# cavelandiah/BBMap

Hardware: AMD Instinct MI355X
Metric: aligned_reads_per_sec (higher is better)
Workload: dtype int32

## Files before the change

bbmap_amd/csrc/mapper_host.hip:

```cpp
#include <hip/hip_runtime.h>

#include <algorithm>
#include <cstdlib>
#include <cstring>
#include <new>
#include <thread>
#include <vector>

#include "mapper_ctx.h"

using namespace bbmapper;

extern "C" int bbmap_default_config_profile(int32_t profile, bbmap_config *c) {
    if (!c || (profile != BBIDX_PROFILE_BBMAP && profile != BBIDX_PROFILE_PACBIO)) return bbfail(BBMAP_E_ARG, "bbmap_default_config: bad argument");
    memset(c, 0, sizeof *c);
    c->paired = 0; c->max_reads = 0; c->max_sites = 32;
    c->extraPadding = 10; c->maxPairDist = 32000; c->averagePairDist = 100; c->maxRescueDist = 1200; c->maxRescueMismatches = 32;
    c->maxTrimSitesToRetain = 800; c->trimList = 1; c->doRescue = 1; c->clearzone3 = 800; c->fastCols = 0; c->jobsPerRead = 0;
    c->finalStage = profile == BBIDX_PROFILE_BBMAP ? 1 : 0;
    if (profile == BBIDX_PROFILE_PACBIO) {
        c->max_read_len = 6016; c->minRatio = 0.46f; c->slowAlignPadding = 8; c->slowRescuePadding = 16; c->tipSearchDist = 15;
        c->alignColumns = 7600; c->msaMaxColumns = 7600;
    } else {
        c->max_read_len = 150; c->minRatio = 0.56f; c->slowAlignPadding = 4; c->slowRescuePadding = 8; c->tipSearchDist = 100;
        c->alignColumns = 3000; c->msaMaxColumns = 3000;
    }
    c->reserved[3] = profile;
    return BBMAP_OK;
}
extern "C" int bbmap_default_config(bbmap_config *c) { return bbmap_default_config_profile(BBIDX_PROFILE_BBMAP, c); }

extern "C" void bbmap_destroy(bbmap_ctx *c) {
    if (!c) return;
    (void)hipSetDevice(c->cfg.device);
    for (void *p : c->allocs) (void)hipFree(p);
    if (c->h_counters) (void)hipHostFree(c->h_counters);
    if (c->tierThread.joinable()) c->tierThread.join();
    if (c->tier) bbmap_destroy(c->tier);
    bbidx_launch_free(&c->probeLs);
    for (DevBuf &b : c->buf) b.release();
    if (c->hostStream) (void)hipStreamDestroy(c->hostStream);
    if (c->tierStream) (void)hipStreamDestroy(c->tierStream);
    if (c->dpStream) (void)hipStreamDestroy(c->dpStream);
    if (c->evFork) (void)hipEventDestroy(c->evFork);
    if (c->evJoin) (void)hipEventDestroy(c->evJoin);
    if (c->ownsMsa && c->msaGapped && c->msaGapped != c->msa) bbmsa_destroy(c->msaGapped);
    if (c->ownsMsa && c->msa) bbmsa_destroy(c->msa);
    for (hipEvent_t e : c->ev) if (e) (void)hipEventDestroy(e);
    delete c;
}

static int create_impl(bbidx_ctx *index, const bbmap_config *cfg, bbmap_ctx *parent, bbmap_ctx **out) {
    if (!index || !cfg || !out) return bbfail(BBMAP_E_ARG, "bbmap_create: null argument");
    *out = nullptr;
    const int profile = cfg->reserved[3];
    if (profile != BBIDX_PROFILE_BBMAP && profile != BBIDX_PROFILE_PACBIO) return bbfail(BBMAP_E_ARG, "bbmap_create: unknown profile (bbmap_config.reserved[3])");
    if (profile != index->dev.p.profile) return bbfail(BBMAP_E_ARG, "bbmap_create: the index was built for the other profile (BBIDX_PROFILE_*)");
    const bool pacbio = profile == BBIDX_PROFILE_PACBIO;
    if (cfg->max_reads < 1 || cfg->max_read_len < 1 || cfg->max_read_len > (pacbio ? BBIDX_PACBIO_MAX_READ_LEN : 600))
        return bbfail(BBMAP_E_ARG, "bbmap_create: max_reads >= 1 and max_read_len in 1..600 (1..6016 for BBIDX_PROFILE_PACBIO)");
    if (cfg->max_sites < 1 || cfg->max_sites > BBMAP_MAX_SITES_LIMIT) return bbfail(BBMAP_E_ARG, "bbmap_create: max_sites must be 1..4096");
    if (cfg->paired && (cfg->max_reads & 1)) return bbfail(BBMAP_E_ARG, "bbmap_create: paired mode takes an even number of reads");
    if (cfg->msaMaxColumns < 64 || cfg->msaMaxColumns > (pacbio ? 8192 : 4096)) return bbfail(BBMAP_E_ARG, "bbmap_create: msaMaxColumns must be 64..4096 (..8192 for BBIDX_PROFILE_PACBIO)");
    if (cfg->device != index->device) return bbfail(BBMAP_E_ARG, "bbmap_create: the index lives on another device");
    BBHIP(hipSetDevice(cfg->device));
    bbmap_ctx *c = new (std::nothrow) bbmap_ctx();
    if (!c) return bbfail(BBMAP_E_NOMEM, "bbmap_create: out of host memory");
    c->cfg = *cfg; c->index = index;
    int rc = BBMAP_OK;
    auto bail = [&](int code) { bbmap_destroy(c); return code; };
    if ((rc = bbidx_launch_init(index, &c->probeLs)) != BBMAP_OK) return bail(rc);
    Settings &S = c->S;
    const float R = cfg->minRatio;
    S.minRatio = R;
    { const float a = R * .80f, b = 1.0f - ((1.0f - R) * 1.4f); S.ratioPaired = a > b ? a : b; }
    { const float a = R * .60f, b = 1.0f - ((1.0f - R) * 1.8f); S.ratioPreRescue = a > b ? a : b; }
    S.slowAlignPadding = cfg->slowAlignPadding; S.slowRescuePadding = cfg->slowRescuePadding; S.extraPadding = cfg->extraPadding;
    S.tipSearchDist = cfg->tipSearchDist; S.maxPairDist = cfg->maxPairDist; S.averagePairDist = cfg->averagePairDist;
    S.maxRescueDist = cfg->maxRescueDist; S.maxRescueMismatches = cfg->maxRescueMismatches; S.maxTrimSitesToRetain = cfg->maxTrimSitesToRetain;
    S.trimList = cfg->trimList; S.doRescue = cfg->doRescue; S.alignColumns = cfg->alignColumns; S.clearzone3 = cfg->clearzone3;
    S.maxIndel = index->dev.p.maxIndel; S.paired = cfg->paired; S.rescueSkip = 0;
    if (pacbio) { S.ptsMatch = 90; S.ptsMatch2 = 100; S.ptsSub = -137; S.ptsSub2 = -49; S.ptsSub3 = -25; S.impDelta = -305; }
    else { S.ptsMatch = 70; S.ptsMatch2 = 100; S.ptsSub = -127; S.ptsSub2 = -51; S.ptsSub3 = -25; S.impDelta = -495; }
    S.clearzone1e = 2 * S.ptsMatch2 - S.ptsMatch - S.ptsSub + 1;
    S.msaMaxColumns = cfg->msaMaxColumns;
    if (pacbio) { S.ptsSubR = -157; S.ptsIns = -205; S.ptsIns2 = -42; S.ptsIns3 = -23; S.ptsIns4 = -8; S.ptsDel = -292; S.ptsDel2 = -37; S.ptsDel3 = -17; S.ptsDel4 = -2; }
    else { S.ptsSubR = -147; S.ptsIns = -395; S.ptsIns2 = -39; S.ptsIns3 = -23; S.ptsIns4 = -8; S.ptsDel = -472; S.ptsDel2 = -33; S.ptsDel3 = -9; S.ptsDel4 = -1; }
    S.ptsDel5 = -1; S.ptsGap = -2;
    if (pacbio && (cfg->finalStage < 0 || cfg->finalStage > 2)) return bail(bbfail(BBMAP_E_ARG, "bbmap_create: finalStage must be 0, 1 or 2"));
    S.finalStage = cfg->finalStage ? 1 : 0;
    S.finalPolicy = (pacbio && cfg->finalStage == 1) ? 1 : 0;
    {
        const float rP = S.finalPolicy ? 1.5f : 1.6f, r1 = S.finalPolicy ? 2.2f : 2.0f, r1b = S.finalPolicy ? 2.8f : 2.6f, r1c = S.finalPolicy ? 4.8f : 4.6f;
        const float m2 = (float)S.ptsMatch2;
        S.czP = (int)(rP * m2); S.cz1 = (int)(r1 * m2); S.cz1b = (int)(r1b * m2); S.cz1c = (int)(r1c * m2);
        S.czLimit1e = 40;
    }
    index->dev.p.quitAfterTwoPerfects = cfg->paired ? 0 : 1;
    S.expLimit = (cfg->alignColumns * 17) / 20 - (2 * (cfg->slowAlignPadding + 10));
    const int maxRows = ((cfg->max_read_len + 31) / 32) * 32;
    c->maxRows = maxRows;
    bbmsa_config mc; memset(&mc, 0, sizeof mc);
    mc.device = cfg->device; mc.maxRows = maxRows;
    bbmsa_config gc;
    if (pacbio) {
        mc.maxRows = cfg->max_read_len + 4 > 6100 ? 6100 : cfg->max_read_len + 4;
        c->maxRows = mc.maxRows;
        mc.maxColumns = cfg->msaMaxColumns;
        mc.reserved[2] = BBMSA_SCHEME_9PACBIO;
        gc = mc;
        c->plainColumns = mc.maxColumns;
        if (parent) { c->msa = parent->msa; c->msaGapped = parent->msaGapped; c->ownsMsa = false; }
        else {
            c->ownsMsa = true;
            if ((rc = bbmsa_create(&mc, &c->msa)) != BBMAP_OK) return bail(rc);
            c->msaGapped = c->msa;
        }
    } else {
        mc.maxColumns = cfg->fastCols > 0 ? cfg->fastCols : 256;
        if (mc.maxColumns > cfg->msaMaxColumns) mc.maxColumns = cfg->msaMaxColumns;
        c->plainColumns = mc.maxColumns;
        gc = mc;
        gc.maxColumns = cfg->msaMaxColumns;
        gc.reserved[0] = 32; gc.reserved[1] = 640 < gc.maxColumns ? 640 : gc.maxColumns;
        if (const char *e = getenv("BBMAP_G2_LANES")) { if (*e) gc.reserved[0] = atoi(e); }
        if (const char *e = getenv("BBMAP_G2_COLS")) { if (*e) gc.reserved[1] = atoi(e) < gc.maxColumns ? atoi(e) : gc.maxColumns; }
        (void)parent;
        c->ownsMsa = true;
        if ((rc = bbmsa_create(&mc, &c->msa)) != BBMAP_OK) return bail(rc);
        if ((rc = bbmsa_create(&gc, &c->msaGapped)) != BBMAP_OK) return bail(rc);
    }
    const long long n = cfg->max_reads;
    const int cap = cfg->max_sites;
    c->narrowMinJobs = getenv("BBMAP_NARROW_MIN_JOBS") ? atoll(getenv("BBMAP_NARROW_MIN_JOBS")) : 32768;
    c->sortWide = !(getenv("BBMAP_SORT_WIDE") && atoi(getenv("BBMAP_SORT_WIDE")) == 0);
    if (!pacbio) {
        const long long lat = getenv("BBMAP_LATENCY_JOBS") ? atoll(getenv("BBMAP_LATENCY_JOBS")) : 4096;
        if ((rc = bbmsa_set_latency_jobs(c->msa, lat)) != BBMAP_OK) return bail(rc);
        if (c->msaGapped != c->msa && (rc = bbmsa_set_latency_jobs(c->msaGapped, lat)) != BBMAP_OK) return bail(rc);
    }
    const int jpr = cfg->jobsPerRead > 0 ? cfg->jobsPerRead : 3;
    c->jobCap = n * jpr + 1024;
    c->gjobCap = parent ? n * 16 + 4096 : (n * jpr) / 24 + 4096;
    if (cfg->jobsPerRead < 0) c->jobCap = c->gjobCap = -(long long)cfg->jobsPerRead;
    c->rescCap = parent ? n * 64 + 1024 : n * 2 + 1024;
    c->matchStride = ((maxRows + c->plainColumns + 15) / 16) * 16;
    c->gmatchStride = ((maxRows + gc.maxColumns + 2 + 128 * 8 + 15) / 16) * 16;
#define DA(ptr, count) if ((rc = dalloc(c, &(ptr), (size_t)(count))) != BBMAP_OK) return bail(rc)
    DA(c->d_psites, n * cap); DA(c->d_pnsites, n);
    DA(c->d_ms, n * cap); DA(c->d_mcount, n); DA(c->d_near, n);
    DA(c->d_slow, n);
    DA(c->d_active[0], n); DA(c->d_active[1], n);
    DA(c->d_counters, CNT_WORDS);
    DA(c->d_jobs, c->jobCap); DA(c->d_jinfo, c->jobCap); DA(c->d_results, c->jobCap); DA(c->d_match, c->jobCap * c->matchStride);
    DA(c->d_gjobs, c->gjobCap); DA(c->d_ggaps, c->gjobCap); DA(c->d_ginfo, c->gjobCap); DA(c->d_gresults, c->gjobCap); DA(c->d_gmatch, c->gjobCap * c->gmatchStride);
    DA(c->d_rjobs, c->rescCap); DA(c->d_rinfo, c->rescCap); DA(c->d_rres, c->rescCap); DA(c->d_rsite, c->rescCap);
    DA(c->d_pres, n / 2 + 1);
    if (S.finalStage) {
        c->poolUnits = (n * (long long)(3 * (cfg->max_read_len + 16)) + 65536) / 4;
        if (const char *e = getenv("BBMAP_FINAL_POOL_UNITS")) { if (*e && atoll(e) >= 64) c->poolUnits = atoll(e); }
        DA(c->d_fin, n); DA(c->d_final, n); DA(c->d_pool, c->poolUnits * 4);
    }
    const int nch = index->dev.nchroms;
    DA(c->d_chromMin, nch + 1); DA(c->d_chromOff, nch + 1);
#undef DA
    c->d_chromArr = index->dev.chromArr; c->d_chromArrLen = index->dev.chromArrLen;
    {
        std::vector<const uint8_t *> hc((size_t)nch + 1);
        if (hipMemcpy(hc.data(), index->dev.chromArr, sizeof(void *) * hc.size(), hipMemcpyDeviceToHost) != hipSuccess) return bail(bbfail(BBMAP_E_HIP, "bbmap_create: reading the chromosome table failed"));
        c->refsBase = hc[1];
        std::vector<long long> off((size_t)nch + 1, 0);
        for (int i = 1; i <= nch; i++) off[(size_t)i] = (long long)(hc[(size_t)i] - hc[1]);
        if (hipMemcpy(c->d_chromOff, off.data(), 8 * off.size(), hipMemcpyHostToDevice) != hipSuccess) return bail(bbfail(BBMAP_E_HIP, "bbmap_create: upload failed"));
        if (hipMemset(c->d_chromMin, 0, 4 * ((size_t)nch + 1)) != hipSuccess) return bail(bbfail(BBMAP_E_HIP, "bbmap_create: memset failed"));
    }
    if (hipHostMalloc((void **)&c->h_counters, CNT_WORDS * 4) != hipSuccess) return bail(bbfail(BBMAP_E_NOMEM, "bbmap_create: pinned allocation failed"));
    for (hipEvent_t &e : c->ev) if (hipEventCreate(&e) != hipSuccess) return bail(bbfail(BBMAP_E_HIP, "bbmap_create: hipEventCreate failed"));
    if (!getenv("BBMAP_SERIAL_DP") && !pacbio) {
        if (hipStreamCreateWithFlags(&c->dpStream, hipStreamNonBlocking) != hipSuccess || hipEventCreateWithFlags(&c->evFork, hipEventDisableTiming) != hipSuccess ||
            hipEventCreateWithFlags(&c->evJoin, hipEventDisableTiming) != hipSuccess) return bail(bbfail(BBMAP_E_HIP, "bbmap_create: stream / event creation failed"));
    }
    *out = c;
    return BBMAP_OK;
}

extern "C" int bbmap_create(bbidx_ctx *index, const bbmap_config *cfg, bbmap_ctx **out) {
    bbmap_ctx *c = nullptr;
    BBTRY(create_impl(index, cfg, nullptr, &c));
    if (cfg->reserved[1] >= 0) {
        bbmap_config tc = *cfg;
        long long tn = cfg->reserved[1] > 0 ? cfg->reserved[1] : 4096;
        if (tn > cfg->max_reads) tn = cfg->max_reads;
        if (cfg->paired) tn &= ~1ll;
        tc.max_reads = (int32_t)tn;
        tc.max_sites = cfg->reserved[2] > 0 ? cfg->reserved[2] : 1024;
        tc.jobsPerRead = 128;
        tc.reserved[1] = -1;
        if (tn >= (cfg->paired ? 2 : 1) && tc.max_sites > cfg->max_sites) {
            const int rc = create_impl(index, &tc, c, &c->tier);
            if (rc != BBMAP_OK) { bbmap_destroy(c); return rc; }
            const long long units = cfg->paired ? cfg->max_reads / 2 : cfg->max_reads;
            if (dalloc(c, &c->d_tierUnits, (size_t)units + 1) != BBMAP_OK || dalloc(c, &c->d_tierReads, (size_t)tn) != BBMAP_OK ||
                dalloc(c, &c->d_tierReadIds, (size_t)tn) != BBMAP_OK) { bbmap_destroy(c); return BBMAP_E_NOMEM; }
            if (hipStreamCreateWithFlags(&c->tierStream, hipStreamNonBlocking) != hipSuccess) { bbmap_destroy(c); return bbfail(BBMAP_E_HIP, "bbmap_create: hipStreamCreate failed"); }
        }
    }
    *out = c;
    return BBMAP_OK;
}

static int read_counters(bbmap_ctx *c, hipStream_t stream) {
    BBHIP(hipMemcpyAsync(c->h_counters, c->d_counters, CNT_WORDS * 4, hipMemcpyDeviceToHost, stream));
    BBHIP(hipStreamSynchronize(stream));
    return BBMAP_OK;
}

template <class T> static int regrow(bbmap_ctx *c, hipStream_t stream, T **p, size_t oldCount, size_t newCount, std::vector<void *> &dead) {
    void *d = nullptr;
    if (hipMalloc(&d, (newCount ? newCount : 1) * sizeof(T)) != hipSuccess) return bbfail(BBMAP_E_NOMEM, "bbmap_map_batch_device: growing a fill log failed (device memory)");
    if (oldCount) BBHIP(hipMemcpyAsync(d, *p, oldCount * sizeof(T), hipMemcpyDeviceToDevice, stream));
    for (void *&q : c->allocs) if (q == (void *)*p) q = d;
    dead.push_back((void *)*p);
    *p = (T *)d;
    return BBMAP_OK;
}
struct DeadArrays {
    hipStream_t stream; std::vector<void *> v;
    explicit DeadArrays(hipStream_t s) : stream(s) {}
    ~DeadArrays() { if (!v.empty()) { (void)hipStreamSynchronize(stream); for (void *q : v) (void)hipFree(q); } }
};
static int grow_logs(bbmap_ctx *c, hipStream_t stream, Dev &D, long long needJobs, long long needGapped, long long usedJobs, long long usedGapped) {
    DeadArrays guard(stream);
    std::vector<void *> &dead = guard.v;
    if (needJobs > c->jobCap) {
        long long nc = c->jobCap * 2; if (nc < needJobs) nc = needJobs + needJobs / 4 + 1024;
        BBTRY(regrow(c, stream, &c->d_jobs, (size_t)usedJobs, (size_t)nc, dead));
        BBTRY(regrow(c, stream, &c->d_jinfo, (size_t)usedJobs, (size_t)nc, dead));
        BBTRY(regrow(c, stream, &c->d_results, (size_t)usedJobs, (size_t)nc, dead));
        BBTRY(regrow(c, stream, &c->d_match, (size_t)usedJobs * c->matchStride, (size_t)nc * c->matchStride, dead));
        c->jobCap = nc;
    }
    if (needGapped > c->gjobCap) {
        long long nc = c->gjobCap * 2; if (nc < needGapped) nc = needGapped + needGapped / 4 + 1024;
        BBTRY(regrow(c, stream, &c->d_gjobs, (size_t)usedGapped, (size_t)nc, dead));
        BBTRY(regrow(c, stream, &c->d_ggaps, (size_t)usedGapped, (size_t)nc, dead));
        BBTRY(regrow(c, stream, &c->d_ginfo, (size_t)usedGapped, (size_t)nc, dead));
        BBTRY(regrow(c, stream, &c->d_gresults, (size_t)usedGapped, (size_t)nc, dead));
        BBTRY(regrow(c, stream, &c->d_gmatch, (size_t)usedGapped * c->gmatchStride, (size_t)nc * c->gmatchStride, dead));
        c->gjobCap = nc;
    }
    c->h_counters[CNT_STAGE_FILLS] = (unsigned)usedJobs; c->h_counters[CNT_STAGE_GAPPED] = (unsigned)usedGapped;
    BBHIP(hipMemcpyAsync(c->d_counters + CNT_FILLS, c->h_counters + CNT_STAGE_FILLS, 8, hipMemcpyHostToDevice, stream));
    BBHIP(hipStreamSynchronize(stream));
    D.jobs = c->d_jobs; D.jinfo = c->d_jinfo; D.results = c->d_results; D.match = c->d_match; D.jobCap = c->jobCap;
    D.gjobs = c->d_gjobs; D.ggaps = c->d_ggaps; D.ginfo = c->d_ginfo; D.gresults = c->d_gresults; D.gmatch = c->d_gmatch; D.gjobCap = c->gjobCap;
    c->stats.log_growths += 1.0f;
    return BBMAP_OK;
}

static int run_fills(bbmap_ctx *c, hipStream_t stream, const uint8_t *bases, long long jobBase, long long nNew, long long gBase, long long gNew,
                     bool finalStage = false) {
    bbmsa_use_narrow(c->msa, !finalStage && nNew >= c->narrowMinJobs);
    bbmsa_sort_by_width(c->msa, false);
    if (c->msaGapped != c->msa) { bbmsa_use_narrow(c->msaGapped, false); bbmsa_sort_by_width(c->msaGapped, c->sortWide); }
    hipStream_t gs = (c->dpStream && nNew > 0) ? c->dpStream : stream;
    if (gNew > 0) {
        if (gs != stream) { BBHIP(hipEventRecord(c->evFork, stream)); BBHIP(hipStreamWaitEvent(gs, c->evFork, 0)); }
        BBTRY(bbmsa_align_gapped_batch_device(c->msaGapped, gs, gNew, c->d_gjobs + gBase, c->d_ggaps + gBase, bases, c->refsBase,
                                             c->d_gresults + gBase, c->d_gmatch + gBase * c->gmatchStride, c->gmatchStride));
        if (gs != stream) { BBHIP(hipEventRecord(c->evJoin, gs)); if (nNew > 0) BBTRY(bbmsa_wait_first_pass(c->msaGapped, stream)); }
    }
    if (nNew > 0)
        BBTRY(bbmsa_align_batch_device(c->msa, stream, nNew, c->d_jobs + jobBase, bases, c->refsBase, c->d_results + jobBase,
                                      c->d_match + jobBase * c->matchStride, c->matchStride));
    const int r1 = nNew > 0 ? bbmsa_last_route_flags(c->msa) : 0;
    const int r2 = gNew > 0 ? bbmsa_last_route_flags(c->msaGapped) : 0;
    c->stats.dp_narrow_launches += (r1 & 1) + (r2 & 1);
    c->stats.dp_sorted_launches += ((r1 >> 1) & 1) + ((r2 >> 1) & 1);
    if (gNew > 0 && gs != stream) BBHIP(hipStreamWaitEvent(stream, c->evJoin, 0));
    return BBMAP_OK;
}

static void add_dp_ms(bbmap_ctx *c, bool plain, bool gapped) {
    float k3[3];
    if (plain && bbmsa_last_kernel_ms3(c->msa, k3) == BBMAP_OK) { c->stats.ms_dp_narrow += k3[0]; c->stats.ms_dp_wave += k3[1]; c->stats.ms_dp_generic += k3[2];
                                                                 if (k3[1] > c->stats.ms_dp_wave_max) c->stats.ms_dp_wave_max = k3[1]; }
    if (gapped && c->msaGapped != c->msa && bbmsa_last_kernel_ms3(c->msaGapped, k3) == BBMAP_OK) c->stats.ms_dp_gapped += k3[0] + k3[1] + k3[2];
    static const bool show = getenv("BBMAP_DP_COUNTS") != nullptr;
    if (show) {
        int64_t n4[4];
        if (plain && bbmsa_last_counts(c->msa, n4) == BBMAP_OK)
            fprintf(stderr, "dp counts plain : narrow finished %lld, narrow handed on %lld, wavefront list %lld, to the wide/generic pass %lld\n",
                    (long long)n4[0], (long long)n4[1], (long long)n4[2], (long long)n4[3]);
        if (gapped && bbmsa_last_counts(c->msaGapped, n4) == BBMAP_OK)
            fprintf(stderr, "dp counts second: narrow finished %lld, narrow handed on %lld, wavefront list %lld, to the wide/generic pass %lld\n",
                    (long long)n4[0], (long long)n4[1], (long long)n4[2], (long long)n4[3]);
    }
}

static void tier_start_async(bbmap_ctx *c, long long found);

struct Rounds {
    bool finalStage;
    long long jobBase, gBase;
    long long nActive;
    int cur = 0;
    bool first = true, ranPlain = false, ranGapped = false;
};
template <class K> static int round_begin(bbmap_ctx *c, hipStream_t stream, Dev &D, Rounds &R, K kernel) {
    BBHIP(hipMemsetAsync(c->d_counters + CNT_NEXT_ACTIVE, 0, 4, stream));
    if (R.finalStage) {
        BBHIP(hipMemsetAsync(c->d_counters + CNT_POOL_AT_FAILURE, 0xff, 4, stream));
        BBHIP(hipMemsetAsync(c->d_counters + CNT_POOL_FAILED, 0, 4, stream));
    }
    D.activeIn = R.first ? nullptr : c->d_active[R.cur]; D.nActiveIn = (int)R.nActive; D.activeOut = c->d_active[1 - R.cur];
    BBTRY(launch<128>(kernel, R.nActive, stream, D));
    return read_counters(c, stream);
}
static int round_end(bbmap_ctx *c, hipStream_t stream, Dev &D, Rounds &R, const uint8_t *bases) {
    add_dp_ms(c, R.ranPlain, R.ranGapped);
    const long long asked = c->h_counters[CNT_FILLS], gasked = c->h_counters[CNT_GAPPED_FILLS];
    const long long total = asked < c->jobCap ? asked : c->jobCap, gtotal = gasked < c->gjobCap ? gasked : c->gjobCap;
    BBTRY(run_fills(c, stream, bases, R.jobBase, total - R.jobBase, R.gBase, gtotal - R.gBase, R.finalStage));
    R.ranPlain = total > R.jobBase; R.ranGapped = gtotal > R.gBase;
    R.jobBase = total; R.gBase = gtotal;
    if (asked > c->jobCap || gasked > c->gjobCap) BBTRY(grow_logs(c, stream, D, asked, gasked, total, gtotal));
    R.nActive = c->h_counters[CNT_NEXT_ACTIVE];
    R.cur = 1 - R.cur; R.first = false;
    return BBMAP_OK;
}

static int grow_pool(bbmap_ctx *c, hipStream_t stream, Dev &D, long long used, long long units, bool setCounter) {
    if (units > 0x7ffffff0LL) return bbfail(BBMAP_E_NOMEM, "bbmap_map_batch_device: the final stage's match strings exceed 8 GB; map smaller batches");
    DeadArrays guard(stream);
    BBTRY(regrow(c, stream, &c->d_pool, (size_t)used * 4, (size_t)units * 4, guard.v));
    if (setCounter) {
        c->h_counters[CNT_STAGE_POOL] = (unsigned)used;
        BBHIP(hipMemcpyAsync(c->d_counters + CNT_POOL_UNITS, c->h_counters + CNT_STAGE_POOL, 4, hipMemcpyHostToDevice, stream));
    }
    BBHIP(hipStreamSynchronize(stream));
    c->poolUnits = units; D.pool = c->d_pool; D.poolUnits = units;
    return BBMAP_OK;
}

static int run_final_stage(bbmap_ctx *c, hipStream_t stream, Dev &D, int64_t n_reads, const uint8_t *bases, long long jobBase, long long gBase,
                           long long &finalRounds, long long &finalLocal) {
    const long long units = c->cfg.paired ? n_reads / 2 : n_reads;
    const unsigned *h = c->h_counters;
    D.fin = c->d_fin; D.finalOut = c->d_final; D.pool = c->d_pool; D.poolUnits = c->poolUnits;
    D.match = c->d_match; D.gmatch = c->d_gmatch; D.matchStride = c->matchStride; D.gmatchStride = c->gmatchStride;
    BBTRY(launch<128>(final_begin_kernel, units, stream, D));
    Rounds R; R.finalStage = true; R.jobBase = jobBase; R.gBase = gBase; R.nActive = n_reads;
    for (int round = 0; R.nActive > 0; round++) {
        if (round > 64 * c->cfg.max_sites + 64) return bbfail(BBMAP_E_HIP, "bbmap_map_batch_device: the final stage does not come to an end (internal error)");
        BBTRY(round_begin(c, stream, D, R, final_round_kernel));
        BBTRY(round_end(c, stream, D, R, bases));
        if (h[CNT_POOL_FAILED] > 0) {
            const long long used = h[CNT_POOL_AT_FAILURE];
            long long nu = c->poolUnits * 2, need = used + ((long long)h[CNT_POOL_UNITS] - used) * 2 + 65536;
            if (nu < need) nu = need;
            BBTRY(grow_pool(c, stream, D, used, nu, true));
        }
        finalRounds++;
    }
    BBHIP(hipStreamSynchronize(stream));
    add_dp_ms(c, R.ranPlain, R.ranGapped);
    BBHIP(hipMemsetAsync(c->d_counters + CNT_LOCAL_READS, 0, 8, stream));
    BBTRY(launch<128>(final_end_kernel, units, stream, D));
    BBTRY(read_counters(c, stream));
    finalLocal = h[CNT_LOCAL_READS];
    const long long used = h[CNT_POOL_UNITS], local = h[CNT_LOCAL_UNITS];
    if (used + local + 64 > c->poolUnits) BBTRY(grow_pool(c, stream, D, used, used + local + 65536, false));
    BBTRY(launch<128>(final_local_kernel, units, stream, D));
    return BBMAP_OK;
}


static void fill_dev(bbmap_ctx *c, Dev &D, int64_t n_reads, const bbidx_read *reads, uint8_t *bases, int64_t minus_delta) {
    memset(&D, 0, sizeof D);
    D.S = c->S; D.reads = reads; D.bases = bases; D.minusDelta = minus_delta; D.nreads = n_reads;
    D.chromArr = c->d_chromArr; D.chromArrLen = c->d_chromArrLen; D.refsBase = c->refsBase;
    D.psites = c->d_psites; D.pnsites = c->d_pnsites; D.maxSites = c->cfg.max_sites;
    D.ms = c->d_ms; D.mcount = c->d_mcount; D.cap = c->cfg.max_sites; D.nearArr = c->d_near; D.slow = c->d_slow;
    D.counters = c->d_counters; D.plainColumns = c->plainColumns; D.fillAhead = c->cfg.reserved[0] ? 0 : 1;
    D.jobs = c->d_jobs; D.jinfo = c->d_jinfo; D.results = c->d_results; D.jobCap = c->jobCap;
    D.gjobs = c->d_gjobs; D.ggaps = c->d_ggaps; D.ginfo = c->d_ginfo; D.gresults = c->d_gresults; D.gjobCap = c->gjobCap;
    D.rjobs = c->d_rjobs; D.rinfo = c->d_rinfo; D.rres = c->d_rres; D.pres = c->d_pres; D.rescCap = c->rescCap; D.rsite = c->d_rsite;
    if (c->index->scafFilter) D.scaf = c->index->scaf;
}

static int finish_stats(bbmap_ctx *c, hipStream_t stream, bool whole, long long fillsBefore, long long finalRounds, long long finalLocal) {
    BBHIP(hipEventRecord(c->ev[EV_FINAL_END], stream));
    BBTRY(read_counters(c, stream));
    const unsigned *h = c->h_counters;
    const hipEvent_t *ev = c->ev;
    c->poolUsed = 4ll * h[CNT_POOL_UNITS];
    c->nJobs = h[CNT_FILLS]; c->nGapped = h[CNT_GAPPED_FILLS];
    c->finalFills = c->S.finalStage ? (c->nJobs + c->nGapped) - fillsBefore : 0;
    bbmap_stats &st = c->stats;
    st.fills = c->nJobs; st.gapped_fills = c->nGapped;
    (void)hipEventElapsedTime(&st.ms_final, ev[EV_RESCUE_END], ev[EV_FINAL_END]);
    if (whole) {
        st.reads_overflowed = h[CNT_OVERFLOWED]; st.reads_without_site = h[CNT_NO_SITE];
        st.refills = h[CNT_REFILLS]; st.rescue_fills = h[CNT_RESCUE_FILLS]; st.fills_dropped = h[CNT_FILLS_DROPPED];
        st.sites_cross_scaffold = h[CNT_CROSS_SCAFFOLD];
        (void)hipEventElapsedTime(&st.ms_probe, ev[EV_START], ev[EV_PROBE_END]);
        (void)hipEventElapsedTime(&st.ms_begin, ev[EV_PROBE_END], ev[EV_BEGIN_END]);
        (void)hipEventElapsedTime(&st.ms_score, ev[EV_BEGIN_END], ev[EV_SCORE_END]);
        (void)hipEventElapsedTime(&st.ms_slow, ev[EV_SCORE_END], ev[EV_SLOW_END]);
        (void)hipEventElapsedTime(&st.ms_finish, ev[EV_SLOW_END], ev[EV_FINISH_END]);
        (void)hipEventElapsedTime(&st.ms_rescue, ev[EV_FINISH_END], ev[EV_RESCUE_END]);
        (void)hipEventElapsedTime(&st.ms_total, ev[EV_START], ev[EV_FINAL_END]);
    } else st.ms_total = st.ms_final;
    st.final_fills = c->finalFills; st.final_rounds = finalRounds; st.final_local = finalLocal;
    return BBMAP_OK;
}

static int map_records(bbmap_ctx *c, hipStream_t stream, int64_t n_reads, const bbidx_read *reads, uint8_t *bases,
                       int64_t minus_delta, const int8_t *baseScores, const int32_t *keyinfo, bool writeRc) {
    memset(&c->stats, 0, sizeof c->stats);
    c->stats.reads = n_reads;
    BBHIP(hipMemsetAsync(c->d_counters, 0, CNT_WORDS * 4, stream));
    BBHIP(hipEventRecord(c->ev[EV_START], stream));
    BBTRY(bbidx_find_batch_device_with(c->index, &c->probeLs, stream, n_reads, reads, bases, baseScores, keyinfo, c->d_psites, c->cfg.max_sites,
                                      c->d_pnsites, writeRc ? bases + minus_delta : nullptr));
    if (writeRc) BBTRY(launch<128>(revcomp_unprobed_kernel, n_reads, stream, reads, (long long)n_reads, (int)c->index->dev.p.k, (const uint8_t *)bases, bases + minus_delta));
    BBHIP(hipEventRecord(c->ev[EV_PROBE_END], stream));
    Dev D;
    fill_dev(c, D, n_reads, reads, bases, minus_delta);
    const long long units = c->cfg.paired ? n_reads / 2 : n_reads;
    BBTRY(launch<128>(begin_kernel, units, stream, D));
    if (c->tier) {
        BBTRY(launch<128>(collect_overflow_kernel, units, stream, c->d_mcount, units, c->cfg.paired, c->d_tierUnits, c->d_counters + CNT_TIER_FOUND));
    }
    BBHIP(hipEventRecord(c->ev[EV_BEGIN_END], stream));
    BBTRY(launch<128>(score_kernel, n_reads, stream, D));
    BBHIP(hipEventRecord(c->ev[EV_SCORE_END], stream));
    Rounds R; R.finalStage = false; R.jobBase = R.gBase = 0; R.nActive = n_reads;
    for (int round = 0; R.nActive > 0 && round < 4 * c->cfg.max_sites + 4; round++) {
        BBTRY(round_begin(c, stream, D, R, slow_round_kernel));
        if (round == 0) {
            float pms = 0; long long ps[5];
            if (writeRc && bbidx_last_stats_with(c->index, &c->probeLs, (int64_t *)ps, &pms) == BBMAP_OK) for (int i = 0; i < 5; i++) c->stats.probe_stats[i] = ps[i];
            c->overAfterBegin = c->h_counters[CNT_OVERFLOWED];
            if (c->tier && c->h_counters[CNT_TIER_FOUND] > 0 && c->tier->msa != c->msa) tier_start_async(c, c->h_counters[CNT_TIER_FOUND]);
        }
        BBTRY(round_end(c, stream, D, R, bases));
        c->stats.rounds++;
    }
    long long jobBase = R.jobBase, gBase = R.gBase;
    BBHIP(hipEventRecord(c->ev[EV_SLOW_END], stream));
    BBTRY(launch<128>(finish_kernel, n_reads, stream, D));
    BBHIP(hipEventRecord(c->ev[EV_FINISH_END], stream));
    if (c->cfg.paired && c->cfg.doRescue) {
        const long long pairs = n_reads / 2;
        for (int pass = 0; pass < 2; pass++) {
            D.pass = pass;
            BBHIP(hipMemsetAsync(c->d_counters + CNT_RESCUE_SEARCHES, 0, 4, stream));
            BBTRY(launch<128>(rescue_plan_kernel, pairs, stream, D));
            BBTRY(read_counters(c, stream));
            const long long nsearch = c->h_counters[CNT_RESCUE_SEARCHES];
            if (nsearch > c->rescCap) return bbfail(BBMAP_E_NOMEM, "bbmap_map_batch_device: rescue list full");
            c->stats.rescue_scans += nsearch;
            if (nsearch == 0) {
                BBTRY(launch<128>(rescue_finish_kernel, pairs, stream, D));
                continue;
            }
            hipEvent_t q0 = c->ev[EV_QUICK_BEGIN], q1 = c->ev[EV_QUICK_END];
            BBHIP(hipEventRecord(q0, stream));
            BBTRY(bbpipe_quick_rescue_device(stream, nsearch, c->d_rjobs, bases, (const int64_t *)c->d_chromOff, c->d_chromArrLen, c->d_chromMin, c->refsBase,
                                            c->d_rres, c->S.ptsMatch, c->S.ptsMatch2, 1, 100));
            BBHIP(hipEventRecord(q1, stream));
            if (jobBase + nsearch > c->jobCap || gBase + nsearch > c->gjobCap) BBTRY(grow_logs(c, stream, D, jobBase + nsearch, gBase + nsearch, jobBase, gBase));
            BBTRY(launch<128>(rescue_prep_kernel, pairs, stream, D));
            BBTRY(read_counters(c, stream));
            { float ms = 0; if (hipEventElapsedTime(&ms, q0, q1) == hipSuccess) c->stats.ms_quick_rescue += ms; }
            const long long total = c->h_counters[CNT_FILLS], gtotal = c->h_counters[CNT_GAPPED_FILLS];
            if (total > c->jobCap || gtotal > c->gjobCap) return bbfail(BBMAP_E_HIP, "bbmap_map_batch_device: rescue fills beyond the reserved log entries (internal error)");
            BBTRY(run_fills(c, stream, bases, jobBase, total - jobBase, gBase, gtotal - gBase));
            const bool ranPlain = total > jobBase, ranGapped = gtotal > gBase;
            jobBase = total; gBase = gtotal;
            BBTRY(launch<128>(rescue_finish_kernel, pairs, stream, D));
            BBHIP(hipStreamSynchronize(stream));
            add_dp_ms(c, ranPlain, ranGapped);
        }
    }
    BBHIP(hipEventRecord(c->ev[EV_RESCUE_END], stream));
    c->finalFills = 0; c->poolUsed = 0;
    long long finalRounds = 0, finalLocal = 0;
    if (c->S.finalStage) BBTRY(run_final_stage(c, stream, D, n_reads, bases, jobBase, gBase, finalRounds, finalLocal));
    BBTRY(finish_stats(c, stream, true, jobBase + gBase, finalRounds, finalLocal));
    c->ran = true;
    return BBMAP_OK;
}

static int tier_pass(bbmap_ctx *c, hipStream_t s, long long found) {
    bbmap_ctx *t = c->tier;
    const bbmap_ctx::BatchArgs &B = c->batch;
    const int paired = c->cfg.paired;
    c->tierReads = 0; t->ran = false;
    std::vector<int> ids((size_t)found);
    BBHIP(hipMemcpyAsync(ids.data(), c->d_tierUnits, 4 * (size_t)found, hipMemcpyDeviceToHost, s));
    BBHIP(hipStreamSynchronize(s));
    std::sort(ids.begin(), ids.end());
    const long long room = paired ? t->cfg.max_reads / 2 : t->cfg.max_reads;
    const long long take = found < room ? found : room;
    BBHIP(hipMemcpyAsync(c->d_tierUnits, ids.data(), 4 * (size_t)take, hipMemcpyHostToDevice, s));
    BBTRY(launch<128>(gather_reads_kernel, take, s, B.reads, c->d_tierUnits, (int)take, paired, c->d_tierReads, c->d_tierReadIds));
    BBHIP(hipStreamSynchronize(s));
    const long long tn = paired ? 2 * take : take;
    BBTRY(map_records(t, s, tn, c->d_tierReads, B.bases, B.minus_delta, B.baseScores, B.keyinfo, false));
    c->tierReads = tn;
    return BBMAP_OK;
}

static void tier_start_async(bbmap_ctx *c, long long found) {
    c->tierStarted = true; c->tierRc = BBMAP_OK; c->tierErr[0] = 0;
    c->tierThread = std::thread([c, found]() {
        int rc = hipSetDevice(c->cfg.device) == hipSuccess ? BBMAP_OK : BBMAP_E_HIP;
        if (rc == BBMAP_OK) rc = tier_pass(c, c->tierStream, found);
        if (rc != BBMAP_OK) { snprintf(c->tierErr, sizeof c->tierErr, "overflow tier: %s", bbmap_last_error()); }
        c->tierRc = rc;
    });
}

static int tier_finish(bbmap_ctx *c, hipStream_t stream) {
    bbmap_ctx *t = c->tier;
    const long long tn = c->tierReads;
    if (tn == 0) return BBMAP_OK;
    BBHIP(hipMemsetAsync(c->d_counters + CNT_TIER_RESOLVED, 0, 4, stream));
    BBTRY(launch<128>(mark_tier_kernel, tn, stream, c->d_mcount, t->d_mcount, c->d_tierReadIds, (int)tn, c->d_counters + CNT_TIER_RESOLVED));
    BBTRY(read_counters(c, stream));
    bbmap_stats &st = c->stats; const bbmap_stats &ts = t->stats;
    st.reads_reprobed = tn;
    st.reads_overflowed -= (long long)c->h_counters[CNT_TIER_RESOLVED];
    st.reads_without_site += ts.reads_without_site;
    st.fills += ts.fills; st.gapped_fills += ts.gapped_fills; st.refills += ts.refills; st.rescue_scans += ts.rescue_scans;
    st.rescue_fills += ts.rescue_fills; st.fills_dropped += ts.fills_dropped;
    st.final_fills += ts.final_fills; st.final_local += ts.final_local;
    st.dp_narrow_launches += ts.dp_narrow_launches; st.dp_sorted_launches += ts.dp_sorted_launches;
    st.sites_cross_scaffold += ts.sites_cross_scaffold;
    if (getenv("BBMAP_TIER_DEBUG"))
        fprintf(stderr, "[bbmap tier] reads %lld: probe %.2f begin %.2f score %.2f slow %.2f (rounds %lld) finish %.2f rescue %.2f total %.2f\n",
                tn, ts.ms_probe, ts.ms_begin, ts.ms_score, ts.ms_slow, (long long)ts.rounds, ts.ms_finish, ts.ms_rescue, ts.ms_total);
    return BBMAP_OK;
}

static int rescue_skip_rule(bbmap_ctx *c, bool *skip) {
    *skip = false;
    if (!c->d_runStats) return BBMAP_OK;
    bbmap_runstats rs;
    BBHIP(hipStreamSynchronize(c->statsStream));
    BBHIP(hipMemcpy(&rs, c->d_runStats, sizeof rs, hipMemcpyDeviceToHost));
    *skip = rs.mappedRetained2 > 1000 && rs.numMated * 20LL < rs.mappedRetained2;
    return BBMAP_OK;
}

static int adapt_after_batch(bbmap_ctx *c, hipStream_t stream) {
    if (!(c->adaptive & BBMAP_ADAPT_INSERT_LENGTH)) return BBMAP_OK;
    bbmap_runstats rs;
    BBHIP(hipMemcpyAsync(&rs, c->d_runStats, sizeof rs, hipMemcpyDeviceToHost, stream));
    BBHIP(hipStreamSynchronize(stream));
    const bool heldPaired = rs.numMated > c->numMatedSeen;
    c->numMatedSeen = rs.numMated;
    if (rs.numMated > 1000 && heldPaired) {
        volatile float sum = (float)rs.innerLengthSum, cnt = (float)rs.numMated;
        const float q = sum * 1.0f / cnt;
        const int v = (int)q;
        if (v >= 0) BBTRY(bbmap_set_average_pair_dist(c, v));
    }
    return BBMAP_OK;
}

extern "C" int bbmap_get_adaptive_state(bbmap_ctx *c, int32_t *averagePairDist, int32_t *rescueSkipped) {
    if (!c) return bbfail(BBMAP_E_ARG, "bbmap_get_adaptive_state: null context");
    if (averagePairDist) *averagePairDist = c->cfg.averagePairDist;
    if (rescueSkipped) {
        bool skip = false;
        if (c->adaptive & BBMAP_ADAPT_RESCUE_SKIP) { BBHIP(hipSetDevice(c->cfg.device)); BBTRY(rescue_skip_rule(c, &skip)); }
        *rescueSkipped = skip ? 1 : 0;
    }
    return BBMAP_OK;
}

static int map_batch_device(bbmap_ctx *c, hipStream_t stream, int64_t n_reads, const bbidx_read *reads, uint8_t *bases,
                            int64_t minus_delta, const int8_t *baseScores, const int32_t *keyinfo) {
    c->batch = {n_reads, reads, bases, minus_delta, baseScores, keyinfo};
    c->tierStarted = false; c->tierReads = 0;
    if (c->tier) c->tier->ran = false;
    const int rc = map_records(c, stream, n_reads, reads, bases, minus_delta, baseScores, keyinfo, true);
    hipEvent_t e0 = c->ev[EV_TIER_BEGIN], e1 = c->ev[EV_TIER_END];
    if (c->tierStarted) {
        c->tierThread.join();
        if (rc == BBMAP_OK && c->tierRc != BBMAP_OK) return bbfail(c->tierRc, "%s", c->tierErr);
    }
    BBTRY(rc);
    if (c->tier) BBHIP(hipEventRecord(e0, stream));
    if (!c->tier || c->stats.reads_overflowed == 0) return BBMAP_OK;
    if (c->stats.reads_overflowed > c->overAfterBegin || !c->tierStarted) {
        const long long units = c->cfg.paired ? n_reads / 2 : n_reads;
            BBHIP(hipMemsetAsync(c->d_counters + CNT_TIER_FOUND, 0, 4, stream));
        BBTRY(launch<128>(collect_overflow_kernel, units, stream, c->d_mcount, units, c->cfg.paired, c->d_tierUnits, c->d_counters + CNT_TIER_FOUND));
        BBTRY(read_counters(c, stream));
        if (c->h_counters[CNT_TIER_FOUND] > 0) BBTRY(tier_pass(c, stream, c->h_counters[CNT_TIER_FOUND]));
    }
    BBTRY(tier_finish(c, stream));
    BBHIP(hipEventRecord(e1, stream));
    BBHIP(hipStreamSynchronize(stream));
    (void)hipEventElapsedTime(&c->stats.ms_overflow, e0, e1);
    c->stats.ms_total += c->stats.ms_overflow;
    return BBMAP_OK;
}

extern "C" int bbmap_map_batch_device(bbmap_ctx *c, void *stream_, int64_t n_reads, const bbidx_read *reads, uint8_t *bases,
                                      int64_t minus_delta, const int8_t *baseScores, const int32_t *keyinfo) {
    if (!c) return bbfail(BBMAP_E_ARG, "bbmap_map_batch_device: null context");
    if (n_reads < 0 || n_reads > c->cfg.max_reads) return bbfail(BBMAP_E_ARG, "bbmap_map_batch_device: more reads than the context was made for");
    if (c->cfg.paired && (n_reads & 1)) return bbfail(BBMAP_E_ARG, "bbmap_map_batch_device: paired mode takes an even number of reads");
    if (n_reads == 0) { c->ran = false; c->truthNext = nullptr; return BBMAP_OK; }
    if (!reads || !bases || !baseScores || !keyinfo) return bbfail(BBMAP_E_ARG, "bbmap_map_batch_device: null buffer");
    hipStream_t stream = (hipStream_t)stream_;
    BBHIP(hipSetDevice(c->cfg.device));
    c->statsCounted = false;
    const bbmap_truth *truth = c->truthNext;
    c->truthNext = nullptr;
    bool skip = false;
    if (c->adaptive & BBMAP_ADAPT_RESCUE_SKIP) BBTRY(rescue_skip_rule(c, &skip));
    c->S.rescueSkip = skip ? 1 : 0;
    if (c->tier) c->tier->S.rescueSkip = c->S.rescueSkip;
    BBTRY(map_batch_device(c, stream, n_reads, reads, bases, minus_delta, baseScores, keyinfo));
    if (c->adaptive && c->S.finalStage) {
        BBTRY(bbmap_add_run_stats(c, stream, truth));
        BBTRY(adapt_after_batch(c, stream));
    }
    return BBMAP_OK;
}

extern "C" int bbmap_final_batch_device(bbmap_ctx *c, void *stream_, int64_t n_reads, const bbidx_read *reads, uint8_t *bases, int64_t minus_delta,
                                        const bbmap_msite *sites, const int32_t *nsites) {
    if (!c) return bbfail(BBMAP_E_ARG, "bbmap_final_batch_device: null context");
    if (!c->S.finalStage) return bbfail(BBMAP_E_ARG, "bbmap_final_batch_device: the context was created without the final stage");
    if (n_reads < 1 || n_reads > c->cfg.max_reads || (c->cfg.paired && (n_reads & 1))) return bbfail(BBMAP_E_ARG, "bbmap_final_batch_device: bad read count");
    if (!reads || !bases || !sites || !nsites) return bbfail(BBMAP_E_ARG, "bbmap_final_batch_device: null buffer");
    hipStream_t stream = (hipStream_t)stream_;
    BBHIP(hipSetDevice(c->cfg.device));
    c->tierStarted = false; c->tierReads = 0;
    if (c->tier) c->tier->ran = false;
    c->statsCounted = false;
    memset(&c->stats, 0, sizeof c->stats);
    c->stats.reads = n_reads;
    c->batch = {n_reads, reads, bases, minus_delta, nullptr, nullptr};
    BBHIP(hipMemsetAsync(c->d_counters, 0, CNT_WORDS * 4, stream));
    BBHIP(hipMemsetAsync(c->d_slow, 0, sizeof(SlowState) * (size_t)n_reads, stream));
    BBHIP(hipMemcpyAsync(c->d_ms, sites, sizeof(bbmap_msite) * (size_t)n_reads * (size_t)c->cfg.max_sites, hipMemcpyDeviceToDevice, stream));
    BBHIP(hipMemcpyAsync(c->d_mcount, nsites, 4 * (size_t)n_reads, hipMemcpyDeviceToDevice, stream));
    BBHIP(hipEventRecord(c->ev[EV_RESCUE_END], stream));
    Dev D;
    fill_dev(c, D, n_reads, reads, bases, minus_delta);
    long long finalRounds = 0, finalLocal = 0;
    BBTRY(run_final_stage(c, stream, D, n_reads, bases, 0, 0, finalRounds, finalLocal));
    BBTRY(finish_stats(c, stream, false, 0, finalRounds, finalLocal));
    c->ran = true;
    return BBMAP_OK;
}
```

bbmap_amd/csrc/msa_common.h:

```cpp
#pragma once
#include <hip/hip_runtime.h>
#include <stdint.h>
#include "bbmap_amd.h"

namespace bbmsa {

constexpr int kScoreOffset = 11;
constexpr int kTimeMask = 0x7FF;
constexpr int kScoreMask = (int)0xFFFFF800;
constexpr int kMaxTime = 2047;

#define BBMSA_PT(x) ((x) * 2048)
constexpr int P_MATCH = BBMSA_PT(70), P_MATCH2 = BBMSA_PT(100);
constexpr int P_SUB = BBMSA_PT(-127), P_SUBR = BBMSA_PT(-147), P_SUB2 = BBMSA_PT(-51), P_SUB3 = BBMSA_PT(-25);
constexpr int P_INS = BBMSA_PT(-395), P_INS2 = BBMSA_PT(-39), P_INS3 = BBMSA_PT(-23), P_INS4 = BBMSA_PT(-8);
constexpr int P_DEL = BBMSA_PT(-472), P_DEL2 = BBMSA_PT(-33), P_DEL3 = BBMSA_PT(-9), P_DEL4 = BBMSA_PT(-1),
              P_DEL5 = BBMSA_PT(-1);
constexpr int P_DEL_REF_N = BBMSA_PT(-10), P_GAP = BBMSA_PT(-2);
constexpr int kBadOff = (-(((1 << 20) - 1) - 2000) - 1) * 2048;
constexpr int kMinOffScore = (-(((1 << 20) - 1) - 2000)) * 2048;
constexpr int kNegInf = -(1 << 30);
constexpr int kGapLen = 128;

constexpr int kTableLen = 3072;
__host__ __device__ inline int lds_table_ints(int tableLen) { return 2 * tableLen + 320; }

__host__ __device__ inline int lds_job_ints(int fastCols, int tmpBytes) { return (fastCols + 2) + ((fastCols + 2 + 3) >> 2) + ((tmpBytes + 3) >> 2); }

__host__ __device__ inline int calc_del_off(int len) {
    if (len <= 0) return 0;
    int s = P_DEL;
    if (len > 80) { s += ((len - 80 + 3) / 4) * P_DEL5; len = 80; }
    if (len > 20) { s += (len - 20) * P_DEL4; len = 20; }
    if (len > 5) { s += (len - 5) * P_DEL3; len = 5; }
    if (len > 1) s += (len - 1) * P_DEL2;
    return s;
}
__host__ __device__ inline int calc_ins_cum_off(int len) {
    if (len <= 0) return 0;
    long long s = P_INS;
    int n = len;
    if (n > 20) { s += (long long)(n - 20) * P_INS4; n = 20; }
    if (n > 5) { s += (long long)(n - 5) * P_INS3; n = 5; }
    if (n > 1) s += (long long)(n - 1) * P_INS2;
    return s < kMinOffScore ? kMinOffScore : (int)s;
}

__host__ __device__ inline bool fully_defined(int b) {
    const int u = b & ~32;
    return b < 128 && (u == 'A' || u == 'C' || u == 'G' || u == 'T' || u == 'U');
}

struct Scheme11ts {
    static constexpr int OFF = kScoreOffset, TMASK = kTimeMask, SMASK = kScoreMask, MAXT = kMaxTime;
    static constexpr int MATCH = P_MATCH, MATCH2 = P_MATCH2, SUB = P_SUB, SUBR = P_SUBR, SUB2 = P_SUB2, SUB3 = P_SUB3;
    static constexpr int INS = P_INS, INS2 = P_INS2, INS3 = P_INS3, INS4 = P_INS4;
    static constexpr int DEL = P_DEL, DEL2 = P_DEL2, DEL3 = P_DEL3, DEL4 = P_DEL4, DEL5 = P_DEL5;
    static constexpr int DEL_REF_N = P_DEL_REF_N, GAP = P_GAP;
    static constexpr int BAR_I1 = 2, BAR_D1 = 3;
    static constexpr int BADOFF = kBadOff;
    __host__ __device__ static inline int del_off(int len) { return calc_del_off(len); }
    __host__ __device__ static inline int ins_cum_off(int len) { return calc_ins_cum_off(len); }
    __host__ __device__ static inline int col0(int row) { return calc_ins_cum_off(row); }
};
struct Scheme9PacBio {
    static constexpr int OFF = 9, TMASK = 0x1FF, SMASK = (int)0xFFFFFE00, MAXT = 511;
#define BBMSA_PB(x) ((x) * 512)
    static constexpr int MATCH = BBMSA_PB(90), MATCH2 = BBMSA_PB(100);
    static constexpr int SUB = BBMSA_PB(-137), SUBR = BBMSA_PB(-157), SUB2 = BBMSA_PB(-49), SUB3 = BBMSA_PB(-25);
    static constexpr int INS = BBMSA_PB(-205), INS2 = BBMSA_PB(-42), INS3 = BBMSA_PB(-23), INS4 = BBMSA_PB(-8);
    static constexpr int DEL = BBMSA_PB(-292), DEL2 = BBMSA_PB(-37), DEL3 = BBMSA_PB(-17), DEL4 = BBMSA_PB(-2), DEL5 = BBMSA_PB(-1);
    static constexpr int DEL_REF_N = BBMSA_PB(-10), GAP = BBMSA_PB(-2);
    static constexpr int BAR_I1 = 1, BAR_D1 = 1;
    static constexpr int BADOFF = (-(((1 << 22) - 1) - 2000) - 1) * 512;
#undef BBMSA_PB
    __host__ __device__ static inline int del_off(int len) {
        if (len <= 0) return 0;
        int s = DEL;
        if (len > 80) { s += ((len - 80 + 3) / 4) * DEL5; len = 80; }
        if (len > 20) { s += (len - 20) * DEL4; len = 20; }
        if (len > 5) { s += (len - 5) * DEL3; len = 5; }
        if (len > 1) s += (len - 1) * DEL2;
        return s;
    }
    __host__ __device__ static inline int ins_cum_off(int len) {
        if (len <= 0) return 0;
        int s = INS;
        if (len > 20) { s += (len - 20) * INS4; len = 20; }
        if (len > 5) { s += (len - 5) * INS3; len = 5; }
        if (len > 1) s += (len - 1) * INS2;
        return s;
    }
    __host__ __device__ static inline int col0(int row) {
        if (row <= 0) return 0;
        int s = INS;
        if (row >= 20) { s += (row - 19) * INS4; row = 19; }
        if (row >= 5) { s += (row - 4) * INS3; row = 4; }
        if (row >= 2) s += (row - 1) * INS2;
        return s;
    }
};

__device__ inline long long job_count(long long njobs, const unsigned int *njobs_dev) {
    if (!njobs_dev) return njobs;
    const long long n = (long long)__hip_atomic_load(njobs_dev, __ATOMIC_RELAXED, __HIP_MEMORY_SCOPE_AGENT);
    return n < njobs ? n : njobs;
}

struct FillParams {
    const bbmsa_job *jobs;
    const uint8_t *reads;
    const uint8_t *refs;
    bbmsa_result *results;
    uint8_t *match;
    long long njobs;
    const unsigned int *njobs_dev;
    unsigned int *queue;
    unsigned int *dirbuf;
    long long dir_slot_dwords;
    const int *list;
    const unsigned int *list_count;
    int priority;
    int *slow_list;
    unsigned int *slow_count;
    int match_stride;
    int lanesPerJob;
    int fastCols;
    int tmpBytes;
    int tableLen;
    int maxRows, maxColumns;
    int bandwidth;
    float bandwidthRatio;
    int *planes;
    const long long *plane_off;
    int *limits;
    const long long *limits_off;
};

struct NarrowParams {
    const bbmsa_job *jobs;
    const uint8_t *reads;
    const uint8_t *refs;
    bbmsa_result *results;
    uint8_t *match;
    long long njobs;
    const unsigned int *njobs_dev;
    unsigned int *queue;
    int *fast_list;
    unsigned int *fast_count;
    unsigned long long *dirbuf;
    unsigned int *stats;
    int match_stride;
    int maxRows, maxColumns;
    int bandwidth;
    float bandwidthRatio;
    int maxSlack;
};

struct GenericParams {
    const bbmsa_job *jobs;
    const uint8_t *reads;
    const uint8_t *refs;
    bbmsa_result *results;
    uint8_t *match;
    const int *list;
    const unsigned int *list_count;
    long long njobs;
    const unsigned int *njobs_dev;
    int *matrix;
    int *limits;
    unsigned int *queue;
    int match_stride;
    int maxRows, maxColumns;
    int bandwidth;
    float bandwidthRatio;
};

}
```

bbmap_amd/csrc/msa_ctx.h:

```cpp
#pragma once
#include <hip/hip_runtime.h>

#include "bbmap_amd.h"
#include "host_common.h"

struct bbmsa_ctx {
    bbmsa_config cfg = {};
    int device = 0;
    int numCUs = 0;
    int scheme = 0;
    int G = 0, R = 0, fastCols = 0, tmpBytes = 0, blocks = 0, ldsBytes = 0, tableLen = 0, wideTableLen = 0;
    long long dirSlotDwords = 0;
    unsigned int *d_dir = nullptr;
    unsigned int *d_counters = nullptr;
    DevBuf slowList;
    int genThreads = 0;
    int *d_matrix = nullptr;
    int *d_limits = nullptr;
    int wideR = 0, wideCols = 0, wideTmpBytes = 0, wideBlocks = 0, wideLdsBytes = 0;
    long long wideDirSlotDwords = 0;
    unsigned int *d_wideDir = nullptr;
    DevBuf slowList2;
    int narrowBlocks = 0, narrowSlack = 0;
    bool narrowOff = false;
    bool narrowUsed = false;
    bool lastSorted = false, lastLatency = false, lastIndirect = false;
    bool sortByWidth = false;
    unsigned int *d_widthHist = nullptr;
    long long latencyJobs = 0;
    unsigned long long *d_narrowDir = nullptr;
    DevBuf fastList;
    DevBuf gref, gaux, gjobs;
    hipEvent_t ev[4] = {};
    bool timed = false;
    bool banded = false;
    bool legacyOnly = false;
    struct bbmsa_legacy *legacy = nullptr;
    int stripBlocks = 0, stripLds = 0;
    long long stripDwords = 0, stripSlotDwords = 0;
    int *d_stripBoundary = nullptr;
    uint8_t *d_stripTmp = nullptr;
    int pipeK = 0, pipeSlots = 0, pipeJobsMax = 0;
    int *d_pipeBoundary = nullptr, *d_pipeSync = nullptr;
};

int bbmsa_align_impl(bbmsa_ctx *c, void *stream_, int64_t n_jobs, const uint32_t *n_jobs_dev, const bbmsa_job *jobs,
                     const uint8_t *reads, const uint8_t *refs, bbmsa_result *results, uint8_t *match, int32_t match_stride);

void bbmsa_use_narrow(bbmsa_ctx *c, bool on);
int bbmsa_wait_first_pass(bbmsa_ctx *c, void *waiter);
void bbmsa_sort_by_width(bbmsa_ctx *c, bool on);
int bbmsa_set_latency_jobs(bbmsa_ctx *c, int64_t n);
enum { BBMSA_ROUTE_NARROW = 1, BBMSA_ROUTE_SORTED = 2, BBMSA_ROUTE_LATENCY = 4 };
int bbmsa_last_route_flags(const bbmsa_ctx *c);

int bbmsa_legacy_create(bbmsa_ctx *c);
void bbmsa_legacy_destroy(bbmsa_ctx *c);
```

bbmap_amd/csrc/msa_fill_narrow.hip:

```cpp
#include "msa_common.h"

namespace bbmsa {

namespace {

constexpr int NB = 16;
static_assert(NB == 16, "the sliding reference-byte window (w0/w1/w2) and the 64-bit direction word are laid out for 16 diagonals");

__device__ inline int ctime_n(int t) { return t > kMaxTime ? kMaxTime - 3 : t; }
__device__ inline int del_step_n(int streak) {
    if (streak == 0) return P_DEL;
    if (streak < 5) return P_DEL2;
    if (streak < 20) return P_DEL3;
    if (streak < 80) return P_DEL4;
    return (streak & 3) == 0 ? P_DEL5 : 0;
}
__device__ inline int ins_step_n(int streak) {
    if (streak == 0) return P_INS;
    if (streak < 5) return P_INS2;
    if (streak < 20) return P_INS3;
    return P_INS4;
}
__device__ inline int sub_step_n(int streak) {
    if (streak == 0) return P_SUB;
    if (streak < 5) return P_SUB2;
    return P_SUB3;
}

struct CellOut { int M, D, I; bool good; unsigned nib; };

__device__ inline CellOut cell_eval(int row, int col, int rows, int columns, int call0, int call1, int ref0, int ref1,
                                    int vlimit, int hlimit, int floorv, int subfloor,
                                    int dM, int dD, int dI, int lM, int lD, int uM, int uI) {
    CellOut o;
    const bool gap = ref1 == '-';
    const bool match = (call1 == ref1) & (ref1 != 'N');
    const bool prevMatch = (call0 == ref0) & (ref0 != 'N');
    const int limit = max(vlimit, hlimit);
    const int limit3 = max(floorv, match ? limit - P_MATCH2 : limit - P_SUB3);
    const int delNeeded = max(0, row - col - 1);
    const int insNeeded = max(0, (rows - row) - (columns - col) - 1);
    const int delPen = calc_del_off(delNeeded);
    const int insPen = calc_ins_cum_off(insNeeded);
    bool anyGood = false;
    const int dm = dM & kScoreMask, dd = dD & kScoreMask, di = dI & kScoreMask;
    const int lm = lM & kScoreMask, ld = lD & kScoreMask;
    const int um = uM & kScoreMask, ui = uI & kScoreMask;

    int timeM = 0;
    if (gap | ((dm <= limit3) & (dd <= limit3) & (di <= limit3))) {
        o.M = subfloor;
    } else {
        const int streak = dM & kTimeMask;
        int a, bonus, tA;
        if (match) { a = dm + (prevMatch ? P_MATCH2 : P_MATCH); bonus = P_MATCH; tA = prevMatch ? streak + 1 : 1; }
        else {
            if ((ref1 != 'N') & (call1 != 'N')) a = dm + (prevMatch ? (streak <= 1 ? P_SUBR : P_SUB) : sub_step_n(streak));
            else a = dm;
            bonus = P_SUB; tA = prevMatch ? 1 : streak + 1;
        }
        const int bb = dd + bonus, cc = di + bonus;
        int score, time;
        if ((a >= bb) & (a >= cc)) { score = a; time = tA; }
        else if (bb >= cc) { score = bb; time = 1; }
        else { score = cc; time = 1; }
        const int limit2 = delNeeded > 0 ? limit - delPen : (insNeeded > 0 ? limit - insPen : limit);
        if (score >= limit2) anyGood = true; else score = subfloor;
        timeM = time;
        o.M = score | ctime_n(time);
    }
    bool aWinsD = true;
    if (((lm <= limit) & (ld <= limit)) | (row < 3) | (row > rows - 3)) {
        o.D = subfloor;
    } else {
        const int streak = lD & kTimeMask;
        int a = lm + P_DEL, bsc = ld + del_step_n(streak);
        if (ref1 == 'N') { a += P_DEL_REF_N; bsc += P_DEL_REF_N; }
        else if (gap) { a += P_GAP; bsc += P_GAP; }
        int score, time;
        if (a >= bsc) { score = a; time = 1; } else { score = bsc; time = streak + 1; aWinsD = false; }
        int limit2 = limit;
        if (insNeeded > 0) limit2 = limit - insPen;
        else if (delNeeded > 0) limit2 = limit - calc_del_off(time + delNeeded) + calc_del_off(time);
        if (score >= limit2) anyGood = true; else score = subfloor;
        o.D = score | ctime_n(time);
    }
    bool aWinsI = true;
    if (gap | ((um <= limit) & (ui <= limit)) | ((row < 2) & (col > 1)) | ((row > rows - 2) & (col < columns - 1))) {
        o.I = subfloor;
    } else {
        const int streak = uI & kTimeMask;
        const int a = um + P_INS, bsc = ui + ins_step_n(streak);
        int score, time;
        if (a >= bsc) { score = a; time = 1; } else { score = bsc; time = streak + 1; aWinsI = false; }
        int limit2 = limit;
        if (delNeeded > 0) limit2 = limit - delPen;
        else if (insNeeded > 0) limit2 = limit - calc_ins_cum_off(time + insNeeded) + calc_ins_cum_off(time);
        if (score >= limit2) anyGood = true; else score = subfloor;
        o.I = score | ctime_n(time);
    }
    const bool msStay = (timeM > 1) | (dm >= max(dd, di));
    const unsigned nibM = msStay ? 0u : ((dd >= di) ? 1u : 2u);
    o.nib = nibM | (aWinsD ? 0u : 4u) | (aWinsI ? 0u : 8u);
    o.good = anyGood;
    return o;
}

}

#ifndef BBMSA_NARROW_OCC
#define BBMSA_NARROW_OCC 2
#endif
__global__ __launch_bounds__(64, BBMSA_NARROW_OCC) void msa_fill_narrow_kernel(const NarrowParams p) {
    const int lane = threadIdx.x;
    unsigned long long *dirw = p.dirbuf + (long long)blockIdx.x * (long long)(p.maxRows + 1) * 64;
    const bool ctxBanded = !(p.bandwidth < 1 && p.bandwidthRatio <= 0.0f);
    unsigned nDone = 0, nLeft = 0;
    const long long NJ = job_count(p.njobs, p.njobs_dev);

    for (;;) {
        long long j = -1;
        bbmsa_job jb;
        jb.read_off = 0; jb.ref_off = 0; jb.read_len = 0; jb.ref_len = 0; jb.refStartLoc = 0; jb.refEndLoc = -1; jb.minScore = 0; jb.flags = 0;
        int rows = 0, a = 0, b = -1, columns = 0, minScore = 0, mode = 0;
        for (;;) {
            const long long q = (long long)atomicAdd(p.queue, 1u);
            if (q >= NJ) break;
            const bbmsa_job t = p.jobs[q];
            int ta = t.refStartLoc, tb = t.refEndLoc;
            const int tmode = t.flags & BBMSA_MODE_MASK;
            if (t.flags & BBMSA_CLAMP_WINDOW) {
                ta = max(0, ta); tb = min(t.ref_len - 1, tb);
                if (tb - ta >= p.maxColumns) tb = min(t.ref_len - 1, ta + p.maxColumns - 1);
            }
            const int trows = t.read_len, tcols = tb - ta + 1;
            bool cand = !ctxBanded && trows >= NB && tcols >= trows && trows <= p.maxRows && tcols <= p.maxColumns &&
                        tmode != BBMSA_FILL_UNLIMITED_RAW;
            int tmin = t.minScore;
            if (cand && tmode == BBMSA_FILL_LIMITED) {
                if (tmin < 1 || (tcols + trows < 90) || (tcols > trows + min(170, trows + 20))) cand = false;
                else tmin -= 120;
            }
            if (cand && (70 + 100 * (trows - 1)) - tmin > p.maxSlack) cand = false;
            if (cand) { j = q; jb = t; rows = trows; a = ta; b = tb; columns = tcols; minScore = tmin; mode = tmode; break; }
            const unsigned k = atomicAdd(p.fast_count, 1u);
            p.fast_list[k] = (int)q;
        }
        if (!__any(j >= 0)) break;
        bool active = j >= 0;
        const uint8_t *rd = p.reads + jb.read_off;
        const uint8_t *rf = p.refs + jb.ref_off + a;
        const int D0 = (columns - rows) / 2 - NB / 2;

        const int maxGain = (rows - 1) * P_MATCH2 + P_MATCH;
        const int minScoreOff = minScore * 2048;
        const int floorv = minScoreOff - maxGain;
        const int subfloor = floorv - 5 * P_MATCH2;

        int vs = 0;
        if (active) {
            bool allDef = true;
            for (int c = 0; c < columns; c++) allDef = allDef && fully_defined(rf[c]);
            bool nextDef = false;
            for (int i = rows - 1; i >= 0; i--) {
                const bool def = fully_defined(rd[i]);
                vs += def ? (nextDef ? P_MATCH2 : P_MATCH) : 0;
                nextDef = def;
            }
            if (!allDef) { active = false; const unsigned k = atomicAdd(p.fast_count, 1u); p.fast_list[k] = (int)j; nLeft++; }
        }
        auto hlimit_at = [&](int col) -> int {
            const int hs = col <= columns - 1 ? P_MATCH + (columns - 1 - col) * P_MATCH2 : 0;
            return max(minScoreOff - hs, floorv);
        };

        int aM[NB + 1], aD[NB + 1], aI[NB + 1];
#pragma unroll
        for (int i = 0; i <= NB; i++) { aM[i] = 0; aD[i] = 0; aI[i] = 0; }
        long long iters = 0;
        int prevMin = 1, prevMax = columns;
        int stoppedRow = INT_MAX;
        int lastColStart = 1, lastHasGood = 0;
        int bestM = 0, bestD = 0, bestI = 0, bestMc = -1, bestDc = -1, bestIc = -1;
        unsigned long long w0 = 0, w1 = 0, w2 = 0;
        auto ref_col = [&](int c) -> unsigned { return (active && c >= 1 && c <= columns) ? (unsigned)rf[c - 1] : 0u; };
        if (active) {
            for (int k = 0; k < 8; k++) w0 |= (unsigned long long)ref_col(1 + D0 - 1 + k) << (8 * k);
            for (int k = 0; k < 8; k++) w1 |= (unsigned long long)ref_col(1 + D0 - 1 + 8 + k) << (8 * k);
            for (int k = 0; k < 2; k++) w2 |= (unsigned long long)ref_col(1 + D0 - 1 + 16 + k) << (8 * k);
        }
        int call0 = '?';
        int maxRowsBatch = active ? rows : 0;
        for (int d = 32; d >= 1; d >>= 1) maxRowsBatch = max(maxRowsBatch, __shfl_xor(maxRowsBatch, d, 64));

        for (int row = 1; row <= maxRowsBatch; row++) {
            const bool rowAct = active && row <= rows && stoppedRow == INT_MAX;
            if (!__any(rowAct)) break;
            int call1 = 0;
            bool enter = false;
            int colStart = 0, colStop = 0, vlimit = 0;
            if (rowAct) {
                call1 = rd[row - 1];
                colStart = prevMin; colStop = prevMax;
                enter = !(colStart < 0 || colStop < colStart);
                if (!enter) stoppedRow = row;
                const bool def = fully_defined(call1);
                const bool nextDef = row < rows ? fully_defined(rd[row]) : false;
                vs -= def ? (nextDef ? P_MATCH2 : P_MATCH) : 0;
                vlimit = max(minScoreOff - vs, floorv);
            }
            const int c0 = row + D0;
            bool go = rowAct && enter;
            if (go && row == 1) {
                bool outGood = false;
                for (int c = 1; c <= columns; c++) {
                    if (c >= c0 && c < c0 + NB) continue;
                    const int ref1 = rf[c - 1], ref0 = c < 2 ? '!' : rf[c - 2];
                    const CellOut o = cell_eval(1, c, rows, columns, call0, call1, ref0, ref1, vlimit, hlimit_at(c), floorv, subfloor,
                                                0, 0, 0, c == 1 ? calc_ins_cum_off(1) : subfloor, c == 1 ? calc_ins_cum_off(1) : subfloor, 0, 0);
                    outGood = outGood || o.good;
                }
                iters += (long long)(columns - max(0, min(columns, c0 + NB - 1) - max(1, c0) + 1));
                if (outGood) go = false;
            }
            if (go && row > 1 && (colStart < c0 || colStart > c0 + NB - 1)) go = false;
            const bool bailEarly = rowAct && enter && !go;
            int minGood = -1, maxGood = -2;
            bool rowDone = false;
            int leftM = subfloor, leftD = subfloor;
            if (go && colStart == 1) { leftM = calc_ins_cum_off(row); leftD = leftM; }
            unsigned long long word = 0;
            const int insPrev = calc_ins_cum_off(row - 1);
            const bool lastRow = row == rows;
#pragma unroll
            for (int i = 0; i < NB; i++) {
                const int c = c0 + i;
                const bool inRow = go && c >= colStart && c >= 1 && c <= columns && !rowDone;
                int nM = subfloor, nD = subfloor, nI = subfloor;
                if (inRow) {
                    const unsigned rb0 = (unsigned)((i < 8 ? (w0 >> (8 * (i & 7))) : (w1 >> (8 * (i & 7)))) & 255u);
                    const int k1 = i + 1;
                    const unsigned rb1 = (unsigned)((k1 < 8 ? (w0 >> (8 * (k1 & 7))) : (k1 < 16 ? (w1 >> (8 * (k1 & 7))) : (w2 >> (8 * (k1 & 7))))) & 255u);
                    const int ref0 = c < 2 ? '!' : (int)rb0, ref1 = (int)rb1;
                    const int dM = (c == 1) ? insPrev : aM[i], dD = (c == 1) ? insPrev : aD[i], dI = (c == 1) ? insPrev : aI[i];
                    const int uM = (i + 1 < NB) ? aM[i + 1] : (row == 1 ? 0 : subfloor);
                    const int uI = (i + 1 < NB) ? aI[i + 1] : (row == 1 ? 0 : subfloor);
                    const CellOut o = cell_eval(row, c, rows, columns, call0, call1, ref0, ref1, vlimit, hlimit_at(c), floorv, subfloor,
                                                dM, dD, dI, leftM, leftD, uM, uI);
                    nM = o.M; nD = o.D; nI = o.I;
                    iters++;
                    if (o.good) { maxGood = c; if (minGood < 0) minGood = c; }
                    if (c > colStop && maxGood < c) rowDone = true;
                    word |= (unsigned long long)o.nib << (4 * i);
                    if (lastRow) {
                        if (bestMc < 0 || (nM & kScoreMask) > (bestM & kScoreMask)) { bestM = nM; bestMc = c; }
                        if (bestDc < 0 || (nD & kScoreMask) > (bestD & kScoreMask)) { bestD = nD; bestDc = c; }
                        if (bestIc < 0 || (nI & kScoreMask) > (bestI & kScoreMask)) { bestI = nI; bestIc = c; }
                    }
                    leftM = nM; leftD = nD;
                }
                if (rowAct) { aM[i] = nM; aD[i] = nD; aI[i] = nI; }
            }
            const bool unfinished = go && row > 1 && !rowDone && (c0 + NB - 1 < columns);
            if (bailEarly || unfinished) {
                active = false;
                const unsigned k = atomicAdd(p.fast_count, 1u);
                p.fast_list[k] = (int)j;
                nLeft++;
            } else if (go) {
                prevMin = minGood; prevMax = maxGood;
                dirw[(long long)row * 64 + lane] = word;
                if (lastRow) { lastColStart = colStart; lastHasGood = minGood >= 0; }
            }
            {
                const unsigned nb = ref_col(row + 1 + D0 - 1 + NB + 1);
                w0 = (w0 >> 8) | (w1 << 56);
                w1 = (w1 >> 8) | (w2 << 56);
                w2 = (w2 >> 8) | ((unsigned long long)nb << 8);
            }
            call0 = call1;
        }

        int bScore = INT_MIN, bCol = -1, bState = 0, bPacked = 0;
        if (bestMc >= 0) { bScore = bestM & kScoreMask; bCol = bestMc; bState = 0; bPacked = bestM; }
        if (bestDc >= 0 && (bestD & kScoreMask) > bScore) { bScore = bestD & kScoreMask; bCol = bestDc; bState = 1; bPacked = bestD; }
        if (bestIc >= 0 && (bestI & kScoreMask) > bScore) { bScore = bestI & kScoreMask; bCol = bestIc; bState = 2; bPacked = bestI; }
        int res1, res2, res3, res4 = 0;
        bool fillNull = false;
        if (stoppedRow <= rows) { res1 = 1; res2 = 0; res3 = kBadOff; res4 = 1; fillNull = true; }
        else if (!lastHasGood) { res1 = max(1, lastColStart - 1); res2 = 0; res3 = subfloor; res4 = 1; fillNull = true; }
        else if (bScore < minScoreOff) { res1 = bCol; res2 = bState; res3 = bScore; res4 = 1; fillNull = true; }
        else { res1 = bCol; res2 = bState; res3 = bScore >> kScoreOffset; }

        asm volatile("s_waitcnt vmcnt(0)" ::: "memory");

        if (active) {
            bbmsa_result r;
            r.result[0] = rows; r.result[1] = res1; r.result[2] = res2; r.result[3] = res3; r.result[4] = res4;
            r.status = (fillNull && mode == BBMSA_FILL_LIMITED) ? BBMSA_ST_NULL : BBMSA_ST_OK;
            r.iterations = iters;
            for (int i = 0; i < 8; i++) r.score[i] = 0;
            r.score_len = 0; r.match_len = 0; r.fill_kind = 0; r.columns = columns;
            if (!fillNull && (jb.flags & (BBMSA_DO_SCORE | BBMSA_DO_TRACEBACK))) {
                const bool wantTrace = (jb.flags & BBMSA_DO_TRACEBACK) && p.match != nullptr;
                uint8_t *out = wantTrace ? p.match + j * (long long)p.match_stride : nullptr;
                int row = rows, col = res1, state = res2, n = 0, gaps = 0, stateTime = 0;
                bool overflow = false;
                while (row > 0 && col > 0) {
                    const int i = col - row - D0;
                    unsigned nib = 0;
                    if (i >= 0 && i < NB) nib = (unsigned)(__hip_atomic_load(&dirw[(long long)row * 64 + lane], __ATOMIC_RELAXED, __HIP_MEMORY_SCOPE_AGENT) >> (4 * i)) & 15u;
                    int prev;
                    uint8_t sym;
                    if (state == 0) {
                        prev = (int)(nib & 3u);
                        const int cb = rd[row - 1], rb = rf[col - 1];
                        sym = (cb == rb) ? 'm' : ((!fully_defined(cb) || !fully_defined(rb)) ? 'N' : 'S');
                        row--; col--;
                    } else if (state == 1) {
                        prev = (nib & 4u) ? 1 : 0;
                        const int rb = rf[col - 1];
                        if (rb == '-') { sym = '-'; gaps++; } else sym = 'D';
                        col--;
                    } else {
                        prev = (nib & 8u) ? 2 : 0;
                        sym = (col >= columns) ? 'Y' : 'I';
                        row--;
                    }
                    if (wantTrace) { if (n < p.match_stride) out[n] = sym; else overflow = true; }
                    n++;
                    if (state == prev) stateTime++; else stateTime = 0;
                    state = prev;
                }
                if (jb.flags & BBMSA_DO_SCORE) {
                    int colS = col;
                    if (row > colS) colS -= row;
                    const int bestRefStart = a + colS, bestRefStop = a + res1 - 1;
                    int padLeft = 0, padRight = 0;
                    if (bestRefStart < a) padLeft = max(0, a - bestRefStart);
                    else if (bestRefStart == a && state == 2) padLeft = stateTime;
                    const int bW = (jb.flags & BBMSA_INTERNAL_GAPPED) ? jb.ref_len : b;
                    if (bestRefStop > bW) padRight = max(0, bestRefStop - bW);
                    else if (bestRefStop == bW && res2 == 2) padRight = bPacked & kTimeMask;
                    r.score[0] = bScore >> kScoreOffset; r.score[1] = bestRefStart; r.score[2] = bestRefStop;
                    r.score[3] = rows; r.score[4] = res1; r.score[5] = res2;
                    if (padLeft > 0 || padRight > 0) { r.score[6] = padLeft; r.score[7] = padRight; r.score_len = 8; }
                    else r.score_len = 6;
                }
                if (wantTrace) {
                    if (col != row) { while (row > 0) { if (n < p.match_stride) out[n] = 'X'; else overflow = true; n++; row--; col--; } }
                    const bool keepGaps = (jb.flags & BBMSA_TRACE_KEEP_GAPS) != 0;
                    const int totalLen = keepGaps ? n : n + gaps * (kGapLen - 1);
                    if (overflow || totalLen > p.match_stride) r.match_len = -1;
                    else {
                        for (int x = 0, y = n - 1; x < y; x++, y--) { const uint8_t t0 = out[x]; out[x] = out[y]; out[y] = t0; }
                        if (gaps > 0 && !keepGaps) {
                            int w = totalLen - 1;
                            for (int x = n - 1; x >= 0; x--) {
                                const uint8_t ch = out[x];
                                if (ch != '-') out[w--] = ch;
                                else for (int g = 0; g < kGapLen; g++) out[w--] = 'D';
                            }
                        }
                        r.match_len = totalLen;
                    }
                }
            }
            p.results[j] = r;
            nDone++;
        }
    }
    if (p.stats) {
        for (int d = 32; d >= 1; d >>= 1) { nDone += __shfl_xor(nDone, d, 64); nLeft += __shfl_xor(nLeft, d, 64); }
        if (lane == 0) { if (nDone) atomicAdd(&p.stats[0], nDone); if (nLeft) atomicAdd(&p.stats[1], nLeft); }
    }
}

}
```

bbmap_amd/csrc/msa_host.hip:

```cpp
#include <hip/hip_runtime.h>

#include <cstdio>
#include <cstdlib>
#include <new>

#include "host_common.h"
#include "msa_common.h"
#include "msa_ctx.h"

namespace bbmsa {
struct StripParams {
    const bbmsa_job *jobs; const uint8_t *reads; const uint8_t *refs; bbmsa_result *results; uint8_t *match;
    long long njobs; const unsigned int *njobs_dev; unsigned int *queue; unsigned int *dirbuf;
    long long dir_slot_dwords, dir_strip_dwords; int *boundary; uint8_t *tmpbuf; int *slow_list; unsigned int *slow_count;
    int match_stride; int maxRows, maxColumns; int bandwidth; float bandwidthRatio;
    int pipeK, pipeSlots; int *pipeBoundary; int *pipeSync; int pipeSpinLimit;
};
int strip_rows_per_lane();
const void *strip_kernel_pacbio();
const void *strip_kernel_pacbio_pipelined();
int strip_pipe_sync_ints(int K);
const void *fast_kernel_for(int R, bool banded);
template <class S> __global__ void msa_fill_generic_kernel(const GenericParams p);
__global__ void msa_fill_narrow_kernel(const NarrowParams p);
}

namespace bbmsa {
constexpr int WIDTH_BUCKETS = 1024;
__device__ inline int job_width_bucket(const bbmsa_job &t, int maxColumns) {
    int a = t.refStartLoc, b = t.refEndLoc;
    if (t.flags & BBMSA_CLAMP_WINDOW) { a = max(0, a); b = min(t.ref_len - 1, b); if (b - a >= maxColumns) b = min(t.ref_len - 1, a + maxColumns - 1); }
    const int cols = max(0, b - a + 1);
    return WIDTH_BUCKETS - 1 - min(WIDTH_BUCKETS - 1, cols >> 3);
}
__global__ void width_hist_kernel(const bbmsa_job *jobs, long long n, int maxColumns, unsigned *hist) {
    const long long i = (long long)blockIdx.x * blockDim.x + threadIdx.x;
    if (i < n) atomicAdd(&hist[job_width_bucket(jobs[i], maxColumns)], 1u);
}
__global__ void width_scan_kernel(unsigned *hist, unsigned *listCount, unsigned n) {
    __shared__ unsigned s[WIDTH_BUCKETS];
    const int t = threadIdx.x;
    s[t] = hist[t];
    __syncthreads();
    for (int d = 1; d < WIDTH_BUCKETS; d <<= 1) { const unsigned v = t >= d ? s[t - d] : 0u; __syncthreads(); s[t] += v; __syncthreads(); }
    hist[t] = s[t] - hist[t];
    if (t == 0) *listCount = n;
}
__global__ void width_scatter_kernel(const bbmsa_job *jobs, long long n, int maxColumns, unsigned *cursor, int *list) {
    const long long i = (long long)blockIdx.x * blockDim.x + threadIdx.x;
    if (i < n) list[atomicAdd(&cursor[job_width_bucket(jobs[i], maxColumns)], 1u)] = (int)i;
}
}

static int setup_wide_pass(bbmsa_ctx *c) {
    if (c->wideBlocks > 0) return BBMAP_OK;
    c->wideR = (c->cfg.maxRows + 63) / 64;
    c->wideCols = c->cfg.maxColumns;
    c->wideTmpBytes = ((64 * c->wideR + c->wideCols + 8) + 3) & ~3;
    const int perJob = bbmsa::lds_job_ints(c->wideCols, c->wideTmpBytes);
    c->wideLdsBytes = (bbmsa::lds_table_ints(c->wideTableLen) + perJob) * 4;
    const void *wfn = bbmsa::fast_kernel_for(c->wideR, c->banded);
    if (wfn && c->wideLdsBytes <= 160 * 1024) {
        if (c->wideLdsBytes > 64 * 1024) BBHIP(hipFuncSetAttribute(wfn, hipFuncAttributeMaxDynamicSharedMemorySize, c->wideLdsBytes));
        int per = 0;
        BBHIP(hipOccupancyMaxActiveBlocksPerMultiprocessor(&per, wfn, 64, c->wideLdsBytes));
        if (per < 1) per = 1;
        if (per > 8) per = 8;
        const long long slotDwords = (long long)(((c->wideCols + 64 - 1) >> 3) + 1) * c->wideR * 64;
        BBHIP(hipMalloc(&c->d_wideDir, (size_t)((long long)c->numCUs * per * slotDwords * 4)));
        c->wideDirSlotDwords = slotDwords;
        c->wideBlocks = c->numCUs * per;
    }
    return BBMAP_OK;
}

extern "C" int bbmsa_create(const bbmsa_config *cfg, bbmsa_ctx **out) {
    if (!cfg || !out) return bbfail(BBMAP_E_ARG, "bbmsa_create: null argument");
    *out = nullptr;
    const int scheme = cfg->reserved[2] & 0xFF;
    const bool legacyOnly = (cfg->reserved[2] & BBMSA_LEGACY_ONLY) != 0;
    if (scheme != BBMSA_SCHEME_11TS && scheme != BBMSA_SCHEME_9PACBIO) return bbfail(BBMAP_E_ARG, "bbmsa_create: unknown scoring scheme");
    if (scheme == BBMSA_SCHEME_11TS && (cfg->maxRows < 1 || cfg->maxRows > 640 || cfg->maxColumns < 1 || cfg->maxColumns > 4096))
        return bbfail(BBMAP_E_ARG, "bbmsa_create: maxRows must be 1..640 and maxColumns 1..4096");
    if (scheme == BBMSA_SCHEME_9PACBIO && (cfg->maxRows < 1 || cfg->maxRows > 6100 || cfg->maxColumns < 1 || cfg->maxColumns > 8192))
        return bbfail(BBMAP_E_ARG, "bbmsa_create: the PacBio scheme takes maxRows 1..6100 and maxColumns 1..8192");
    hipDeviceProp_t prop;
    BBTRY(bb_use_gfx950("bbmsa_create", cfg->device, &prop));

    bbmsa_ctx *c = new (std::nothrow) bbmsa_ctx();
    if (!c) return bbfail(BBMAP_E_NOMEM, "bbmsa_create: out of host memory");
    c->cfg = *cfg;
    c->device = cfg->device;
    c->numCUs = prop.multiProcessorCount;

    c->scheme = scheme;
    c->legacyOnly = legacyOnly;
    struct Guard { bbmsa_ctx *c; ~Guard() { if (c) bbmsa_destroy(c); } } guard{c};
    if (legacyOnly) {
        BBHIP(hipMalloc(&c->d_counters, 64));
        BBHIP(hipMemset(c->d_counters, 0, 64));
        const long long planeInts = (long long)(cfg->maxRows + 1) * (cfg->maxColumns + 2);
        c->genThreads = 1;
        BBHIP(hipMalloc(&c->d_matrix, (size_t)(3 * planeInts * 4)));
        BBHIP(hipMalloc(&c->d_limits, (size_t)((cfg->maxRows + cfg->maxColumns + 4) * 4)));
        for (int i = 0; i < 4; i++) BBHIP(hipEventCreate(&c->ev[i]));
        BBTRY(bbmsa_legacy_create(c));
        guard.c = nullptr;
        *out = c;
        return BBMAP_OK;
    }
    if (scheme != BBMSA_SCHEME_11TS) {
        BBHIP(hipMalloc(&c->d_counters, 64));
        BBHIP(hipMemset(c->d_counters, 0, 64));
        const long long planeInts = (long long)(cfg->maxRows + 1) * (cfg->maxColumns + 2);
        const long long perThread = 3 * planeInts * 4;
        long long budget = (long long)env_int("BBMSA_GENERIC_SCRATCH_MB", 40960) << 20;
        long long threads = budget / perThread;
        if (threads > 4096) threads = 4096;
        threads = (threads / 64) * 64;
        if (threads < 64) return bbfail(BBMAP_E_NOMEM, "bbmsa_create: BBMSA_GENERIC_SCRATCH_MB cannot hold one wavefront of scratch matrices for this maxRows x maxColumns");
        c->genThreads = (int)threads;
        BBHIP(hipMalloc(&c->d_matrix, (size_t)(threads * perThread)));
        BBHIP(hipMalloc(&c->d_limits, (size_t)(threads * (cfg->maxRows + cfg->maxColumns + 4) * 4)));
        {
            const int R = bbmsa::strip_rows_per_lane();
            c->stripLds = (cfg->maxColumns + 2) * 4 + ((cfg->maxColumns + 2 + 7) & ~7);
            const void *kfn = bbmsa::strip_kernel_pacbio();
            if (c->stripLds > 64 * 1024) BBHIP(hipFuncSetAttribute(kfn, hipFuncAttributeMaxDynamicSharedMemorySize, c->stripLds));
            int per = (160 * 1024) / (c->stripLds + 512);
            if (per < 1) per = 1;
            if (per > 8) per = 8;
            c->stripBlocks = c->numCUs * per;
            const int strips = (cfg->maxRows + 64 * R - 1) / (64 * R);
            c->stripDwords = (long long)(((cfg->maxColumns + 64) >> 3) + 1) * R * 64;
            c->stripSlotDwords = c->stripDwords * strips;
            long long dirBudget = (long long)env_int("BBMSA_STRIP_DIR_MB", 32768) << 20;
            while (c->stripBlocks > c->numCUs && (long long)c->stripBlocks * c->stripSlotDwords * 4 > dirBudget) c->stripBlocks -= c->numCUs;
            while (c->stripBlocks > 1 && (long long)c->stripBlocks * c->stripSlotDwords * 4 > dirBudget) c->stripBlocks /= 2;
            {
                const void *kp = bbmsa::strip_kernel_pacbio_pipelined();
                if (c->stripLds > 64 * 1024) BBHIP(hipFuncSetAttribute(kp, hipFuncAttributeMaxDynamicSharedMemorySize, c->stripLds));
                int perP = (160 * 1024) / (c->stripLds + 512);
                if (perP < 1) perP = 1;
                if (perP > 8) perP = 8;
                c->pipeK = strips;
                c->pipeSlots = (c->numCUs * perP) / strips;
                if (c->pipeSlots > c->stripBlocks) c->pipeSlots = c->stripBlocks;
                if (c->pipeSlots > 256) c->pipeSlots = 256;
                c->pipeJobsMax = env_int("BBMSA_STRIP_PIPE_JOBS", 512);
                if (strips < 2 || c->pipeSlots < 1) c->pipeJobsMax = 0;
                if (c->pipeJobsMax > 0) {
                    BBHIP(hipMalloc(&c->d_pipeBoundary, (size_t)((long long)c->pipeSlots * strips * 3 * (cfg->maxColumns + 2) * 4)));
                    BBHIP(hipMalloc(&c->d_pipeSync, (size_t)((long long)c->pipeSlots * bbmsa::strip_pipe_sync_ints(strips) * 4)));
                }
            }
            BBHIP(hipMalloc(&c->d_dir, (size_t)((long long)c->stripBlocks * c->stripSlotDwords * 4)));
            BBHIP(hipMalloc(&c->d_stripBoundary, (size_t)((long long)c->stripBlocks * 6 * (cfg->maxColumns + 2) * 4)));
            BBHIP(hipMalloc(&c->d_stripTmp, (size_t)((long long)c->stripBlocks * (cfg->maxRows + cfg->maxColumns + 8))));
        }
        for (int i = 0; i < 4; i++) BBHIP(hipEventCreate(&c->ev[i]));
        guard.c = nullptr;
        *out = c;
        return BBMAP_OK;
    }
    int G = cfg->reserved[0];
    if (G != 16 && G != 32 && G != 64) {
        G = env_int("BBMSA_LANES_PER_JOB", 0);
        if (G != 16 && G != 32 && G != 64) G = (cfg->maxRows <= 320) ? 32 : 64;
    }
    while (G < 64 && (cfg->maxRows + G - 1) / G > 10) G *= 2;
    c->G = G;
    c->R = (cfg->maxRows + G - 1) / G;
    int fastCols = cfg->reserved[1] > 0 ? cfg->reserved[1] : env_int("BBMSA_FAST_COLS", 0);
    if (fastCols <= 0) fastCols = cfg->maxColumns < 640 ? cfg->maxColumns : 640;
    if (fastCols > cfg->maxColumns) fastCols = cfg->maxColumns;
    c->fastCols = fastCols;
    c->tmpBytes = ((G * c->R + fastCols + 8) + 3) & ~3;
    const int jobsPerWave = 64 / G;
    const int perJobInts = bbmsa::lds_job_ints(fastCols, c->tmpBytes);
    {
        const int side = (cfg->maxColumns > cfg->maxRows ? cfg->maxColumns : cfg->maxRows) + 2;
        c->wideTableLen = (side < 2048 ? side : 2048) + cfg->maxRows + 8;
        const int sideF = (fastCols > cfg->maxRows ? fastCols : cfg->maxRows) + 2;
        c->tableLen = (sideF < 2048 ? sideF : 2048) + cfg->maxRows + 8;
    }
    if (c->tableLen > bbmsa::kTableLen) c->tableLen = bbmsa::kTableLen;
    if (c->wideTableLen > bbmsa::kTableLen) c->wideTableLen = bbmsa::kTableLen;
    c->tableLen = (c->tableLen + 3) & ~3; c->wideTableLen = (c->wideTableLen + 3) & ~3;
    c->ldsBytes = (bbmsa::lds_table_ints(c->tableLen) + 4 * jobsPerWave * perJobInts) * 4;
    if (c->ldsBytes > 160 * 1024) return bbfail(BBMAP_E_ARG, "bbmsa_create: fast-path LDS budget exceeded; lower reserved[1] (fastCols)");

    c->banded = !(cfg->bandwidth < 1 && cfg->bandwidthRatio <= 0.0f);
    const void *kfn = bbmsa::fast_kernel_for(c->R, c->banded);
    if (!kfn) return bbfail(BBMAP_E_ARG, "bbmsa_create: no kernel for this rows-per-lane");
    if (c->ldsBytes > 64 * 1024)
        BBHIP(hipFuncSetAttribute(kfn, hipFuncAttributeMaxDynamicSharedMemorySize, c->ldsBytes));
    int blocksPerCU = 0;
    BBHIP(hipOccupancyMaxActiveBlocksPerMultiprocessor(&blocksPerCU, kfn, 256, c->ldsBytes));
    if (blocksPerCU < 1) blocksPerCU = 1;
    const int capBlocks = env_int("BBMSA_BLOCKS_PER_CU", 0);
    if (capBlocks > 0 && capBlocks < blocksPerCU) blocksPerCU = capBlocks;
    c->blocks = c->numCUs * blocksPerCU;

    const int maxSteps = fastCols + G - 1;
    c->dirSlotDwords = (long long)((maxSteps >> 3) + 1) * c->R * G;
    const long long slots = (long long)c->blocks * 4 * jobsPerWave;
    BBHIP(hipMalloc(&c->d_dir, (size_t)(slots * c->dirSlotDwords * 4)));
    BBHIP(hipMalloc(&c->d_counters, 64));
    BBHIP(hipMemset(c->d_counters, 0, 64));

    const long long planeInts = (long long)(cfg->maxRows + 1) * (cfg->maxColumns + 2);
    const long long perThread = 3 * planeInts * 4;
    long long budget = (long long)env_int("BBMSA_GENERIC_SCRATCH_MB", 2048) << 20;
    long long threads = budget / perThread;
    if (threads > 16384) threads = 16384;
    threads = (threads / 64) * 64;
    if (threads < 64) return bbfail(BBMAP_E_NOMEM, "bbmsa_create: BBMSA_GENERIC_SCRATCH_MB cannot hold one wavefront of scratch matrices for this maxRows x maxColumns");
    c->genThreads = (int)threads;
    BBHIP(hipMalloc(&c->d_matrix, (size_t)(threads * perThread)));
    BBHIP(hipMalloc(&c->d_limits, (size_t)(threads * (cfg->maxRows + cfg->maxColumns + 4) * 4)));
    if (cfg->maxColumns > fastCols) BBTRY(setup_wide_pass(c));
    c->narrowSlack = env_int("BBMSA_NARROW_SLACK", 2000);
    if (!c->banded && env_int("BBMSA_NARROW", 1) != 0) {
        int perCU = 0;
        BBHIP(hipOccupancyMaxActiveBlocksPerMultiprocessor(&perCU, (const void *)bbmsa::msa_fill_narrow_kernel, 64, 0));
        if (perCU < 1) perCU = 1;
        if (perCU > 16) perCU = 16;
        c->narrowBlocks = c->numCUs * perCU;
        BBHIP(hipMalloc(&c->d_narrowDir, (size_t)c->narrowBlocks * (size_t)(cfg->maxRows + 1) * 64 * 8));
    }
    c->sortByWidth = env_int("BBMSA_SORT_BY_WIDTH", 0) != 0;
    { const int lat = env_int("BBMSA_LATENCY_JOBS", 0); if (lat > 0) BBTRY(bbmsa_set_latency_jobs(c, lat)); }
    for (int i = 0; i < 4; i++) BBHIP(hipEventCreate(&c->ev[i]));
    guard.c = nullptr;
    *out = c;
    return BBMAP_OK;
}

extern "C" void bbmsa_destroy(bbmsa_ctx *c) {
    if (!c) return;
    (void)hipSetDevice(c->device);
    bbmsa_legacy_destroy(c);
    if (c->d_dir) (void)hipFree(c->d_dir);
    if (c->d_counters) (void)hipFree(c->d_counters);
    if (c->d_widthHist) (void)hipFree(c->d_widthHist);
    for (DevBuf *b : {&c->slowList, &c->slowList2, &c->fastList, &c->gref, &c->gaux, &c->gjobs}) b->release();
    if (c->d_matrix) (void)hipFree(c->d_matrix);
    if (c->d_limits) (void)hipFree(c->d_limits);
    if (c->d_wideDir) (void)hipFree(c->d_wideDir);
    if (c->d_narrowDir) (void)hipFree(c->d_narrowDir);
    if (c->d_stripBoundary) (void)hipFree(c->d_stripBoundary);
    if (c->d_stripTmp) (void)hipFree(c->d_stripTmp);
    if (c->d_pipeBoundary) (void)hipFree(c->d_pipeBoundary);
    if (c->d_pipeSync) (void)hipFree(c->d_pipeSync);
    for (int i = 0; i < 4; i++) if (c->ev[i]) (void)hipEventDestroy(c->ev[i]);
    delete c;
}

extern "C" int bbmsa_align_batch_device(bbmsa_ctx *c, void *stream_, int64_t n_jobs,
                                        const bbmsa_job *jobs, const uint8_t *reads, const uint8_t *refs,
                                        bbmsa_result *results, uint8_t *match, int32_t match_stride) {
    return bbmsa_align_impl(c, stream_, n_jobs, nullptr, jobs, reads, refs, results, match, match_stride);
}

extern "C" int bbmsa_align_batch_device_indirect(bbmsa_ctx *c, void *stream_, const uint32_t *n_jobs_dev, int64_t max_jobs,
                                                 const bbmsa_job *jobs, const uint8_t *reads, const uint8_t *refs,
                                                 bbmsa_result *results, uint8_t *match, int32_t match_stride) {
    if (!n_jobs_dev) return bbfail(BBMAP_E_ARG, "bbmsa_align_batch_device_indirect: null counter");
    return bbmsa_align_impl(c, stream_, max_jobs, n_jobs_dev, jobs, reads, refs, results, match, match_stride);
}

namespace {
struct Batch {
    int64_t n_jobs; const uint32_t *n_jobs_dev; const bbmsa_job *jobs; const uint8_t *reads, *refs; bbmsa_result *results; uint8_t *match;
    int32_t match_stride;
};
template <class P> void set_batch(P &p, const bbmsa_ctx *c, const Batch &B) {
    p.jobs = B.jobs; p.reads = B.reads; p.refs = B.refs; p.results = B.results; p.match = B.match;
    p.njobs = B.n_jobs; p.njobs_dev = B.n_jobs_dev; p.match_stride = B.match_stride;
    p.maxRows = c->cfg.maxRows; p.maxColumns = c->cfg.maxColumns; p.bandwidth = c->cfg.bandwidth; p.bandwidthRatio = c->cfg.bandwidthRatio;
}
template <class S> int launch_generic(bbmsa_ctx *c, const Batch &B, hipStream_t stream, const int *list, const unsigned int *count) {
    bbmsa::GenericParams gp;
    set_batch(gp, c, B);
    gp.list = list; gp.list_count = count;
    gp.matrix = c->d_matrix; gp.limits = c->d_limits; gp.queue = c->d_counters + 2;
    hipLaunchKernelGGL(bbmsa::msa_fill_generic_kernel<S>, dim3(c->genThreads / 64), dim3(64), 0, stream, gp);
    BBHIP(hipGetLastError());
    BBHIP(hipEventRecord(c->ev[2], stream));
    c->timed = true;
    return BBMAP_OK;
}
}

int bbmsa_align_impl(bbmsa_ctx *c, void *stream_, int64_t n_jobs, const uint32_t *n_jobs_dev,
                     const bbmsa_job *jobs, const uint8_t *reads, const uint8_t *refs,
                     bbmsa_result *results, uint8_t *match, int32_t match_stride) {
    if (!c) return bbfail(BBMAP_E_ARG, "bbmsa_align_batch_device: null context");
    if (n_jobs < 0 || n_jobs > 0x7fffffffLL) return bbfail(BBMAP_E_ARG, "bbmsa_align_batch_device: n_jobs out of range");
    if (n_jobs == 0) return BBMAP_OK;
    if (!jobs || !reads || !refs || !results) return bbfail(BBMAP_E_ARG, "bbmsa_align_batch_device: null buffer");
    if (match && match_stride < 1) return bbfail(BBMAP_E_ARG, "bbmsa_align_batch_device: match_stride must be positive");
    hipStream_t stream = (hipStream_t)stream_;
    BBHIP(hipSetDevice(c->device));
    if (c->legacyOnly) return bbfail(BBMAP_E_ARG, "bbmsa_align_batch_device: this context was created for bbmsa_fill_packed only (BBMSA_LEGACY_ONLY)");
    const Batch B = {n_jobs, n_jobs_dev, jobs, reads, refs, results, match, match_stride};
    const size_t listBytes = (size_t)n_jobs * 4;
    BBHIP(c->slowList.grow(listBytes, 0, &stream));
    int *const slowList = c->slowList.as<int>();
    if (c->scheme != BBMSA_SCHEME_11TS) {
        BBHIP(hipMemsetAsync(c->d_counters, 0, 64, stream));
        c->narrowUsed = false; c->lastSorted = false; c->lastLatency = false; c->lastIndirect = n_jobs_dev != nullptr;
        BBHIP(hipEventRecord(c->ev[0], stream));
        BBHIP(hipEventRecord(c->ev[3], stream));
        bbmsa::StripParams sp;
        set_batch(sp, c, B);
        sp.queue = c->d_counters; sp.dirbuf = c->d_dir; sp.dir_slot_dwords = c->stripSlotDwords; sp.dir_strip_dwords = c->stripDwords;
        sp.boundary = c->d_stripBoundary; sp.tmpbuf = c->d_stripTmp; sp.slow_list = slowList; sp.slow_count = c->d_counters + 1;
        long long sblocks = n_jobs < c->stripBlocks ? n_jobs : c->stripBlocks;
        sp.pipeK = 0; sp.pipeSlots = 0; sp.pipeBoundary = nullptr; sp.pipeSync = nullptr;
        sp.pipeSpinLimit = env_int("BBMSA_PIPE_SPIN_LIMIT", 1 << 21);
        if (sp.pipeSpinLimit < 1) sp.pipeSpinLimit = 1;
        void *sargs[] = {&sp};
        if (!n_jobs_dev && c->pipeJobsMax > 0 && n_jobs <= c->pipeJobsMax) {
            const long long slots = n_jobs < c->pipeSlots ? n_jobs : c->pipeSlots;
            sp.pipeK = c->pipeK; sp.pipeSlots = (int)slots; sp.pipeBoundary = c->d_pipeBoundary; sp.pipeSync = c->d_pipeSync;
            BBHIP(hipMemsetAsync(c->d_pipeSync, 0, (size_t)(slots * bbmsa::strip_pipe_sync_ints(c->pipeK) * 4), stream));
            BBHIP(hipLaunchKernel(bbmsa::strip_kernel_pacbio_pipelined(), dim3((unsigned)(slots * c->pipeK)), dim3(64), sargs, (size_t)c->stripLds, stream));
        } else
        BBHIP(hipLaunchKernel(bbmsa::strip_kernel_pacbio(), dim3((unsigned)sblocks), dim3(64), sargs, (size_t)c->stripLds, stream));
        BBHIP(hipEventRecord(c->ev[1], stream));
        return launch_generic<bbmsa::Scheme9PacBio>(c, B, stream, slowList, c->d_counters + 1);
    }
    if (c->wideBlocks > 0) BBHIP(c->slowList2.grow(listBytes, 0, &stream));
    const bool sortJobs = c->sortByWidth && !n_jobs_dev && n_jobs >= 256 && n_jobs > c->latencyJobs && !(c->narrowBlocks > 0 && !c->narrowOff);
    if (c->narrowBlocks > 0 || sortJobs) BBHIP(c->fastList.grow(listBytes, 0, &stream));
    int *const fastList = c->fastList.as<int>();
    BBHIP(hipMemsetAsync(c->d_counters, 0, 64, stream));
    BBHIP(hipEventRecord(c->ev[0], stream));
    const bool useNarrow = c->narrowBlocks > 0 && !c->narrowOff;
    c->narrowUsed = useNarrow;
    if (useNarrow) {
        bbmsa::NarrowParams np;
        set_batch(np, c, B);
        np.queue = c->d_counters + 3; np.fast_list = fastList; np.fast_count = c->d_counters + 4;
        np.dirbuf = c->d_narrowDir; np.stats = c->d_counters + 5; np.maxSlack = c->narrowSlack;
        long long nb = (n_jobs + 63) / 64;
        if (nb > c->narrowBlocks) nb = c->narrowBlocks;
        hipLaunchKernelGGL(bbmsa::msa_fill_narrow_kernel, dim3((unsigned)nb), dim3(64), 0, stream, np);
        BBHIP(hipGetLastError());
    }
    if (sortJobs) {
        if (!c->d_widthHist) BBHIP(hipMalloc(&c->d_widthHist, bbmsa::WIDTH_BUCKETS * 4));
        BBHIP(hipMemsetAsync(c->d_widthHist, 0, bbmsa::WIDTH_BUCKETS * 4, stream));
        const unsigned sb = (unsigned)((n_jobs + 255) / 256);
        hipLaunchKernelGGL(bbmsa::width_hist_kernel, dim3(sb), dim3(256), 0, stream, jobs, (long long)n_jobs, c->cfg.maxColumns, c->d_widthHist);
        hipLaunchKernelGGL(bbmsa::width_scan_kernel, dim3(1), dim3(bbmsa::WIDTH_BUCKETS), 0, stream, c->d_widthHist, c->d_counters + 4, (unsigned)n_jobs);
        hipLaunchKernelGGL(bbmsa::width_scatter_kernel, dim3(sb), dim3(256), 0, stream, jobs, (long long)n_jobs, c->cfg.maxColumns, c->d_widthHist, fastList);
        BBHIP(hipGetLastError());
    }
    BBHIP(hipEventRecord(c->ev[3], stream));

    bbmsa::FillParams fp = {};
    set_batch(fp, c, B);
    fp.queue = c->d_counters; fp.dirbuf = c->d_dir; fp.dir_slot_dwords = c->dirSlotDwords;
    fp.list = (useNarrow || sortJobs) ? fastList : nullptr; fp.list_count = c->d_counters + 4; fp.priority = 0;
    fp.slow_list = slowList; fp.slow_count = c->d_counters + 1;
    fp.lanesPerJob = c->G; fp.fastCols = c->fastCols; fp.tmpBytes = c->tmpBytes; fp.tableLen = c->tableLen;

    const bool latency = c->wideBlocks > 0 && !n_jobs_dev && !useNarrow && n_jobs <= c->latencyJobs;
    c->lastSorted = sortJobs; c->lastLatency = latency; c->lastIndirect = n_jobs_dev != nullptr;
    const int jobsPerBlock = 4 * (64 / c->G);
    long long blocks = (n_jobs + jobsPerBlock - 1) / jobsPerBlock;
    if (blocks > c->blocks) blocks = c->blocks;
    void *args[] = {&fp};
    if (!latency)
        BBHIP(hipLaunchKernel(bbmsa::fast_kernel_for(c->R, c->banded), dim3((unsigned)blocks), dim3(256), args, (size_t)c->ldsBytes, stream));
    const int *genList = slowList;
    const unsigned int *genCount = c->d_counters + 1;
    if (c->wideBlocks > 0) {
        bbmsa::FillParams wp = fp;
        wp.queue = c->d_counters + 8; wp.dirbuf = c->d_wideDir; wp.dir_slot_dwords = c->wideDirSlotDwords;
        wp.list = slowList; wp.list_count = c->d_counters + 1;
        if (latency) { wp.list = nullptr; wp.list_count = nullptr; }
        wp.slow_list = c->slowList2.as<int>(); wp.slow_count = c->d_counters + 7;
        wp.lanesPerJob = 64; wp.fastCols = c->wideCols; wp.tmpBytes = c->wideTmpBytes; wp.tableLen = c->wideTableLen;
        static const int widePrio = env_int("BBMSA_WIDE_PRIORITY", 2);
        wp.priority = widePrio;
        void *wargs[] = {&wp};
        const long long wblocks = latency && n_jobs < c->wideBlocks ? n_jobs : c->wideBlocks;
        BBHIP(hipLaunchKernel(bbmsa::fast_kernel_for(c->wideR, c->banded), dim3((unsigned)wblocks), dim3(64), wargs, (size_t)c->wideLdsBytes, stream));
        genList = wp.slow_list; genCount = c->d_counters + 7;
    }
    BBHIP(hipEventRecord(c->ev[1], stream));
    return launch_generic<bbmsa::Scheme11ts>(c, B, stream, genList, genCount);
}

void bbmsa_use_narrow(bbmsa_ctx *c, bool on) { if (c) c->narrowOff = !on; }
void bbmsa_sort_by_width(bbmsa_ctx *c, bool on) { if (c) c->sortByWidth = on; }
int bbmsa_set_latency_jobs(bbmsa_ctx *c, int64_t n) {
    if (!c || c->scheme != BBMSA_SCHEME_11TS || c->legacyOnly) return BBMAP_OK;
    BBHIP(hipSetDevice(c->device));
    if (n > 0) BBTRY(setup_wide_pass(c));
    if (n > 0 && !c->slowList2.p) BBHIP(c->slowList2.grow(c->slowList.cap));
    c->latencyJobs = c->wideBlocks > 0 ? n : 0;
    return BBMAP_OK;
}
int bbmsa_wait_first_pass(bbmsa_ctx *c, void *waiter) {
    if (!c || !c->timed) return BBMAP_OK;
    BBHIP(hipStreamWaitEvent((hipStream_t)waiter, c->ev[3], 0));
    return BBMAP_OK;
}

extern "C" int bbmsa_last_kernel_ms(bbmsa_ctx *c, float *ms_fast, float *ms_slow) {
    if (!c || !c->timed) return bbfail(BBMAP_E_ARG, "bbmsa_last_kernel_ms: nothing launched yet");
    BBHIP(hipSetDevice(c->device));
    BBHIP(hipEventSynchronize(c->ev[2]));
    float a = 0, b = 0;
    BBHIP(hipEventElapsedTime(&a, c->ev[0], c->ev[1]));
    BBHIP(hipEventElapsedTime(&b, c->ev[1], c->ev[2]));
    if (ms_fast) *ms_fast = a;
    if (ms_slow) *ms_slow = b;
    return BBMAP_OK;
}

extern "C" int bbmsa_last_kernel_ms3(bbmsa_ctx *c, float *ms3) {
    if (!c || !c->timed || !ms3) return bbfail(BBMAP_E_ARG, "bbmsa_last_kernel_ms3: nothing launched yet");
    BBHIP(hipSetDevice(c->device));
    BBHIP(hipEventSynchronize(c->ev[2]));
    BBHIP(hipEventElapsedTime(&ms3[0], c->ev[0], c->ev[3]));
    BBHIP(hipEventElapsedTime(&ms3[1], c->ev[3], c->ev[1]));
    BBHIP(hipEventElapsedTime(&ms3[2], c->ev[1], c->ev[2]));
    return BBMAP_OK;
}

extern "C" int bbmsa_last_counts(bbmsa_ctx *c, int64_t *counts4) {
    if (!c || !c->timed || !counts4) return bbfail(BBMAP_E_ARG, "bbmsa_last_counts: nothing launched yet");
    BBHIP(hipSetDevice(c->device));
    BBHIP(hipEventSynchronize(c->ev[2]));
    unsigned h[16];
    BBHIP(hipMemcpy(h, c->d_counters, sizeof h, hipMemcpyDeviceToHost));
    counts4[0] = h[5]; counts4[1] = h[6]; counts4[2] = c->narrowUsed ? h[4] : 0; counts4[3] = c->wideBlocks > 0 ? h[7] : h[1];
    if (getenv("BBMAP_DP_COUNTS") && c->wideBlocks > 0) fprintf(stderr, "   (first pass handed %u jobs to the wide pass)\n", h[1]);
    return BBMAP_OK;
}

int bbmsa_last_route_flags(const bbmsa_ctx *c) {
    if (!c || !c->timed) return 0;
    return (c->narrowUsed ? BBMSA_ROUTE_NARROW : 0) | (c->lastSorted ? BBMSA_ROUTE_SORTED : 0) | (c->lastLatency ? BBMSA_ROUTE_LATENCY : 0);
}

extern "C" int bbmsa_last_route(bbmsa_ctx *c, int64_t *route8) {
    if (!c || !c->timed || !route8) return bbfail(BBMAP_E_ARG, "bbmsa_last_route: nothing launched yet");
    BBHIP(hipSetDevice(c->device));
    BBHIP(hipEventSynchronize(c->ev[2]));
    unsigned h[16];
    BBHIP(hipMemcpy(h, c->d_counters, sizeof h, hipMemcpyDeviceToHost));
    const bool wide = c->scheme == BBMSA_SCHEME_11TS && c->wideBlocks > 0;
    route8[0] = c->narrowUsed; route8[1] = c->lastSorted; route8[2] = c->lastLatency; route8[3] = wide; route8[4] = c->lastIndirect;
    route8[5] = h[1]; route8[6] = wide ? h[7] : 0; route8[7] = c->narrowUsed ? h[5] : 0;
    return BBMAP_OK;
}

extern "C" int bbmsa_align_batch(bbmsa_ctx *c, int64_t n_jobs, const bbmsa_job *jobs,
                                 const uint8_t *reads, int64_t reads_bytes,
                                 const uint8_t *refs, int64_t refs_bytes,
                                 bbmsa_result *results, uint8_t *match, int32_t match_stride) {
    if (!c) return bbfail(BBMAP_E_ARG, "bbmsa_align_batch: null context");
    if (n_jobs == 0) return BBMAP_OK;
    if (n_jobs < 0 || !jobs || !reads || !refs || !results || reads_bytes < 0 || refs_bytes < 0)
        return bbfail(BBMAP_E_ARG, "bbmsa_align_batch: bad argument");
    BBHIP(hipSetDevice(c->device));
    for (int64_t i = 0; i < n_jobs; i++) {
        const bbmsa_job &j = jobs[i];
        if (j.read_len < 0 || j.read_off < 0 || j.read_off + j.read_len > reads_bytes)
            return bbfail(BBMAP_E_ARG, "bbmsa_align_batch: a read lies outside the reads buffer");
        if (j.ref_len < 0 || j.ref_off < 0 || j.ref_off + j.ref_len > refs_bytes)
            return bbfail(BBMAP_E_ARG, "bbmsa_align_batch: a reference array lies outside the refs buffer");
        if (!(j.flags & BBMSA_CLAMP_WINDOW) && (j.refStartLoc < 0 || j.refEndLoc >= j.ref_len))
            return bbfail(BBMAP_E_ARG, "bbmsa_align_batch: window outside its reference array (set BBMSA_CLAMP_WINDOW to clamp)");
    }
    DevTmp<bbmsa_job> d_jobs; DevTmp<uint8_t> d_reads, d_refs, d_match; DevTmp<bbmsa_result> d_res;
    BBTRY(d_jobs.upload(jobs, (size_t)n_jobs));
    BBTRY(d_reads.upload(reads, (size_t)reads_bytes));
    BBTRY(d_refs.upload(refs, (size_t)refs_bytes));
    BBTRY(d_res.alloc((size_t)n_jobs));
    if (match) BBTRY(d_match.alloc((size_t)n_jobs * (size_t)match_stride));
    BBHIP(hipMemset(d_res, 0xff, (size_t)n_jobs * sizeof(bbmsa_result)));
    BBTRY(bbmsa_align_batch_device(c, nullptr, n_jobs, d_jobs, d_reads, d_refs, d_res, d_match, match_stride));
    BBHIP(hipStreamSynchronize(nullptr));
    BBHIP(hipMemcpy(results, d_res, (size_t)n_jobs * sizeof(bbmsa_result), hipMemcpyDeviceToHost));
    if (match) BBHIP(hipMemcpy(match, d_match, (size_t)n_jobs * (size_t)match_stride, hipMemcpyDeviceToHost));
    return BBMAP_OK;
}
```

Before: 9.048 million.

## Replace narrow fill kernel with multi-lane banded DP kernel using DPP neighbor exchange

Replaces the one-job-per-lane narrow fill kernel with a banded kernel in which a group of Q lanes cooperates on each job. Lanes exchange neighbor cells through DPP row shifts, penalty tables and read/ref bytes are staged in LDS, and direction nibbles are packed into 32-bit words. Blocks grow to 256 threads and the kernel now also runs during the final stage. This is meant to raise parallelism and cut per-lane serial DP latency and direction-buffer traffic, at the cost of band-limited coverage. Jobs that fall outside the band or that bail out are sent to the fallback fast list.

```diff
diff --git a/bbmap_amd/csrc/mapper_host.hip b/bbmap_amd/csrc/mapper_host.hip
--- a/bbmap_amd/csrc/mapper_host.hip
+++ b/bbmap_amd/csrc/mapper_host.hip
@@ -260,7 +260,7 @@
 
 static int run_fills(bbmap_ctx *c, hipStream_t stream, const uint8_t *bases, long long jobBase, long long nNew, long long gBase, long long gNew,
                      bool finalStage = false) {
-    bbmsa_use_narrow(c->msa, !finalStage && nNew >= c->narrowMinJobs);
+    bbmsa_use_narrow(c->msa, nNew >= c->narrowMinJobs);
     bbmsa_sort_by_width(c->msa, false);
     if (c->msaGapped != c->msa) { bbmsa_use_narrow(c->msaGapped, false); bbmsa_sort_by_width(c->msaGapped, c->sortWide); }
     hipStream_t gs = (c->dpStream && nNew > 0) ? c->dpStream : stream;
diff --git a/bbmap_amd/csrc/msa_common.h b/bbmap_amd/csrc/msa_common.h
--- a/bbmap_amd/csrc/msa_common.h
+++ b/bbmap_amd/csrc/msa_common.h
@@ -148,13 +148,15 @@
     unsigned int *queue;
     int *fast_list;
     unsigned int *fast_count;
-    unsigned long long *dirbuf;
     unsigned int *stats;
     int match_stride;
     int maxRows, maxColumns;
     int bandwidth;
     float bandwidthRatio;
     int maxSlack;
+    unsigned int *dirbuf32;
+    int tableLen;
+    int bandRows;
 };
 
 struct GenericParams {
diff --git a/bbmap_amd/csrc/msa_ctx.h b/bbmap_amd/csrc/msa_ctx.h
--- a/bbmap_amd/csrc/msa_ctx.h
+++ b/bbmap_amd/csrc/msa_ctx.h
@@ -28,7 +28,8 @@
     bool sortByWidth = false;
     unsigned int *d_widthHist = nullptr;
     long long latencyJobs = 0;
-    unsigned long long *d_narrowDir = nullptr;
+    int bandRows = 0, bandLds = 0;
+    unsigned int *d_bandDir = nullptr;
     DevBuf fastList;
     DevBuf gref, gaux, gjobs;
     hipEvent_t ev[4] = {};
diff --git a/bbmap_amd/csrc/msa_fill_band.hip b/bbmap_amd/csrc/msa_fill_band.hip
--- /dev/null
+++ b/bbmap_amd/csrc/msa_fill_band.hip
@@ -0,0 +1,427 @@
+#include "msa_common.h"
+#include "msa_cell.h"
+
+namespace bbmsa {
+
+namespace {
+
+__device__ __forceinline__ int from_left(int x, int fill) { return __builtin_amdgcn_update_dpp(fill, x, 0x138, 0xf, 0xf, false); }
+__device__ __forceinline__ int from_right(int x, int fill) { return __builtin_amdgcn_update_dpp(fill, x, 0x130, 0xf, 0xf, false); }
+
+__device__ __forceinline__ unsigned ld_coherent(const unsigned *p) { return __hip_atomic_load(p, __ATOMIC_RELAXED, __HIP_MEMORY_SCOPE_AGENT); }
+__device__ __forceinline__ unsigned ld_coherent(const uint8_t *p) { return __hip_atomic_load(p, __ATOMIC_RELAXED, __HIP_MEMORY_SCOPE_AGENT); }
+
+struct BandSet {
+    int M[4], D[4], I[4];
+    int rows, columns;
+    int c0off;
+    int minScoreOff, vs;
+    unsigned w;
+    int gprev;
+    int gmask, mprev;
+    int gpass;
+    int bail;
+    int rdOff, rfOff;
+    int slot;
+};
+
+}
+
+#ifndef BBMSA_BAND_OCC
+#define BBMSA_BAND_OCC 4
+#endif
+
+template <int Q>
+__global__ __launch_bounds__(256, BBMSA_BAND_OCC) void msa_fill_band_kernel(const NarrowParams p) {
+    constexpr int B = 4 * Q;
+    constexpr int GROUPS = 64 / Q;
+    constexpr int JOBS = 2 * GROUPS;
+    static_assert(Q == 4 || Q == 8 || Q == 16, "a group is a power of two of lanes, its good bits fit 64");
+    extern __shared__ int lds[];
+    const int TL = p.tableLen;
+    int *delC = lds, *insC = lds + TL, *delExt = lds + 2 * TL, *insExt = delExt + 128;
+    int4 *mTab = reinterpret_cast<int4 *>(delExt + 192);
+    LdsPen pen; pen.delC = delC; pen.insC = insC; pen.delExt = delExt; pen.insExt = insExt; pen.mTab = mTab;
+    for (int i = threadIdx.x; i < TL; i += blockDim.x) { delC[i] = calc_del_off(i); insC[i] = calc_ins_cum_off(i); }
+    for (int i = threadIdx.x; i < 128; i += blockDim.x) delExt[i] = SpelledPen<Scheme11ts>().del_ext(i);
+    if (threadIdx.x < 32) insExt[threadIdx.x] = SpelledPen<Scheme11ts>().ins_ext(threadIdx.x);
+    if (threadIdx.x < 32) {
+        const int st = threadIdx.x & 7, mt = (threadIdx.x >> 3) & 1, pv = threadIdx.x >> 4;
+        const MEntry e = SpelledPen<Scheme11ts>().m_entry(min(st, 5), 0, 0, pv != 0, mt != 0);
+        int4 v; v.x = e.addA; v.y = e.bonus; v.z = e.t3sub; v.w = 0;
+        mTab[threadIdx.x] = v;
+    }
+    __syncthreads();
+
+    const int lane = threadIdx.x & 63, wave = threadIdx.x >> 6;
+    const int q = lane & (Q - 1), grp = lane / Q, groupBase = grp * Q;
+    const int RB = (p.bandRows + 4 + 3) & ~3, FB = (p.bandRows + B + 4 + 3) & ~3;
+    uint8_t *jobLds = reinterpret_cast<uint8_t *>(lds + lds_table_ints(TL)) + (long long)wave * JOBS * (RB + FB);
+    unsigned *dir = p.dirbuf32 + ((long long)blockIdx.x * 4 + wave) * (long long)(p.bandRows + 1) * 128;
+    const long long NJ = job_count(p.njobs, p.njobs_dev);
+    unsigned nDone = 0, nLeft = 0;
+
+    for (;;) {
+        long long myJ = -1;
+        if (lane < JOBS) {
+            for (;;) {
+                const long long t_ = (long long)atomicAdd(p.queue, 1u);
+                if (t_ >= NJ) break;
+                const bbmsa_job t = p.jobs[t_];
+                int ta = t.refStartLoc, tb = t.refEndLoc;
+                const int tmode = t.flags & BBMSA_MODE_MASK;
+                if (t.flags & BBMSA_CLAMP_WINDOW) {
+                    ta = max(0, ta); tb = min(t.ref_len - 1, tb);
+                    if (tb - ta >= p.maxColumns) tb = min(t.ref_len - 1, ta + p.maxColumns - 1);
+                }
+                const int trows = t.read_len, tcols = tb - ta + 1;
+                bool cand = trows >= 16 && tcols >= trows && trows <= p.maxRows && trows <= p.bandRows && tcols <= p.maxColumns &&
+                            tmode != BBMSA_FILL_UNLIMITED_RAW;
+                int tmin = t.minScore;
+                if (cand && tmode == BBMSA_FILL_LIMITED) {
+                    if (tmin < 1 || (tcols + trows < 90) || (tcols > trows + min(170, trows + 20))) cand = false;
+                    else tmin -= 120;
+                }
+                if (cand && (70 + 100 * (trows - 1)) - tmin > p.maxSlack) cand = false;
+                if (cand) { myJ = t_; break; }
+                const unsigned k = atomicAdd(p.fast_count, 1u);
+                p.fast_list[k] = (int)t_;
+            }
+        }
+        if (!__any(myJ >= 0)) break;
+
+        BandSet S[2];
+        long long jobJ[2]; bool jobOk[2];
+#pragma unroll
+        for (int s = 0; s < 2; s++) {
+            const long long j = __shfl(myJ, grp * 2 + s, 64);
+            jobJ[s] = j;
+            bbmsa_job jb;
+            jb.read_off = 0; jb.ref_off = 0; jb.read_len = 0; jb.ref_len = 0; jb.refStartLoc = 0; jb.refEndLoc = -1; jb.minScore = 0; jb.flags = 0;
+            if (j >= 0) jb = p.jobs[j];
+            int a = jb.refStartLoc, b = jb.refEndLoc;
+            if (jb.flags & BBMSA_CLAMP_WINDOW) {
+                a = max(0, a); b = min(jb.ref_len - 1, b);
+                if (b - a >= p.maxColumns) b = min(jb.ref_len - 1, a + p.maxColumns - 1);
+            }
+            const int rows = jb.read_len, columns = b - a + 1;
+            int minScore = jb.minScore;
+            if ((jb.flags & BBMSA_MODE_MASK) == BBMSA_FILL_LIMITED) minScore -= 120;
+            const int D0 = (columns - rows) / 2 - B / 2;
+            const uint8_t *rd = p.reads + jb.read_off, *rf = p.refs + jb.ref_off + a;
+            const int rdOff = (grp * 2 + s) * (RB + FB), rfOff = rdOff + RB;
+            int cost = 0; bool allDef = true;
+#pragma unroll 4
+            for (int i = q; i < rows; i += Q) {
+                const int cb = rd[i];
+                jobLds[rdOff + i] = (uint8_t)cb;
+                if (fully_defined(cb)) cost += (i + 1 < rows && fully_defined(rd[i + 1])) ? P_MATCH2 : P_MATCH;
+            }
+            if (j >= 0)
+#pragma unroll 4
+            for (int k = q; k < rows + B + 1; k += Q) {
+                const int col = k + D0;
+                int v = 0;
+                if (col == 0) v = '!';
+                else if (col >= 1 && col <= columns) { v = rf[col - 1]; allDef = allDef && fully_defined(v); }
+                jobLds[rfOff + k] = (uint8_t)v;
+            }
+            for (int c = 1 + q; c <= columns; c += Q) if (c < 1 + D0 || c > D0 + B) allDef = allDef && fully_defined(rf[c - 1]);
+            int nd = allDef ? 0 : 1;
+            for (int d = 1; d < Q; d <<= 1) { cost += __shfl_xor(cost, d, 64); nd |= __shfl_xor(nd, d, 64); }
+            bool ok = j >= 0 && nd == 0;
+
+            const int minScoreOff = minScore * 2048;
+            const int floorv = minScoreOff - ((rows - 1) * P_MATCH2 + P_MATCH);
+            const int subfloor = floorv - 5 * P_MATCH2;
+            if (ok) {
+                const int cl1 = rd[0];
+                const int c0cost = fully_defined(cl1) ? ((rows > 1 && fully_defined(rd[1])) ? P_MATCH2 : P_MATCH) : 0;
+                const int vlimP = max(minScoreOff - (cost - c0cost), floorv) + 2048;
+                int outGood = 0;
+                for (int c = 1 + q; c <= columns; c += Q) {
+                    if (c >= 1 + D0 && c <= D0 + B) continue;
+                    const int ref1 = rf[c - 1];
+                    const int hs = c <= columns - 1 ? P_MATCH + (columns - 1 - c) * P_MATCH2 : 0;
+                    CellIn ci;
+                    ci.row = 1; ci.c = c; ci.rows = rows; ci.insNeededBase = (columns - c) + 1;
+                    ci.cl1 = cl1; ci.ref1 = ref1; ci.refN = false; ci.gap = false; ci.match = cl1 == ref1; ci.act = true;
+                    ci.refPen = 0; ci.limitP = max(vlimP, max(minScoreOff - hs, floorv) + 2048); ci.floorP = floorv + 2048; ci.subfloor = subfloor;
+                    ci.dgM = 0; ci.dgD = 0; ci.dgI = 0;
+                    ci.lM = c == 1 ? insC[1] : subfloor; ci.lD = ci.lM; ci.upM = 0; ci.upI = 0;
+                    ci.delForce = INT_MAX;
+                    ci.insForce = (c > 1 || (1 > rows - 2 && c < columns - 1)) ? INT_MAX : INT_MIN;
+                    ci.pm8 = 0;
+                    const CellOut co = cell_update<Scheme11ts, false>(pen, ci);
+                    outGood |= (co.goodM | co.goodD | co.goodI) ? 1 : 0;
+                }
+                for (int d = 1; d < Q; d <<= 1) outGood |= __shfl_xor(outGood, d, 64);
+                if (outGood) ok = false;
+            }
+            if (j >= 0 && !ok && q == 0) { const unsigned k = atomicAdd(p.fast_count, 1u); p.fast_list[k] = (int)j; nLeft++; }
+            jobOk[s] = ok;
+
+            const int set = (q & 1) ^ s;
+#pragma unroll
+            for (int x = 0; x < 2; x++) if (x == set) {
+                BandSet &T = S[x];
+                for (int i = 0; i < 4; i++) { T.M[i] = 0; T.D[i] = 0; T.I[i] = 0; }
+                T.rows = ok ? rows : 0; T.columns = columns; T.c0off = D0 + 4 * q;
+                T.minScoreOff = minScoreOff; T.vs = cost;
+                T.w = 0; T.gprev = 1; T.gmask = 0; T.mprev = 0; T.gpass = 0; T.bail = 0;
+                T.rdOff = rdOff; T.rfOff = rfOff; T.slot = s;
+            }
+        }
+        __builtin_amdgcn_fence(__ATOMIC_ACQ_REL, "wavefront");
+        __builtin_amdgcn_wave_barrier();
+#pragma unroll
+        for (int x = 0; x < 2; x++) {
+            BandSet &T = S[x];
+            if (T.rows > 0) for (int i = 0; i < 3; i++) T.w |= (unsigned)jobLds[T.rfOff + 1 + 4 * q + i] << (8 * (i + 1));
+        }
+        int maxRowsWave = max(S[0].rows, S[1].rows);
+        for (int d = 32; d >= 1; d >>= 1) maxRowsWave = max(maxRowsWave, __shfl_xor(maxRowsWave, d, 64));
+
+        const int rowLagX = (q + 1) >> 1, rowLagY = q >> 1;
+        for (int k = 1; k <= maxRowsWave + Q / 2; k++) {
+#pragma unroll
+            for (int x = 0; x < 2; x++) {
+                BandSet &T = S[x];
+                const BandSet &O = S[1 - x];
+                const int row = k - (x == 0 ? rowLagX : rowLagY);
+                int lM = from_left(O.M[3], 0), lD = from_left(O.D[3], 0), gIn = from_left(O.gpass, 0);
+                int uM = from_right(O.M[0], 0), uI = from_right(O.I[0], 0), uG = from_right(O.gmask, 0);
+                const bool rowAct = row >= 1 && row <= T.rows;
+                if (rowAct) {
+                    const int rows = T.rows, columns = T.columns;
+                    const int floorv = T.minScoreOff - ((rows - 1) * P_MATCH2 + P_MATCH);
+                    const int subfloor = floorv - 5 * P_MATCH2, floorP = floorv + 2048;
+                    if (q == 0) { lM = subfloor; lD = subfloor; gIn = 0; }
+                    if (q == Q - 1) { uM = row == 1 ? 0 : subfloor; uI = uM; uG = 0; }
+                    const int cl1 = jobLds[T.rdOff + row - 1];
+                    const int clN = row < rows ? jobLds[T.rdOff + row] : 0;
+                    T.vs -= fully_defined(cl1) ? (fully_defined(clN) ? P_MATCH2 : P_MATCH) : 0;
+                    const int vlimP = max(T.minScoreOff - T.vs, floorv) + 2048;
+                    T.w = (T.w >> 8) | ((unsigned)jobLds[T.rfOff + row + 4 * q + 3] << 24);
+                    const int c0 = row + T.c0off;
+                    const int insRow = insC[row], insPrev = insC[row - 1];
+                    const int delForce = (row < 3 || row > rows - 3) ? INT_MAX : INT_MIN;
+                    const unsigned g5 = (unsigned)T.gmask | (((unsigned)uG & 1u) << 4);
+                    const bool rowOne = row == 1;
+                    unsigned goods = 0, mbits = 0, word = 0;
+                    int leftM = lM, leftD = lD;
+#pragma unroll
+                    for (int i = 0; i < 4; i++) {
+                        const int c = c0 + i;
+                        const int ref1 = (int)((T.w >> (8 * i)) & 255u);
+                        const bool inRange = (c >= 1) & (c <= columns);
+                        const bool started = (T.gprev != 0) | ((g5 & ((4u << i) - 1u)) != 0u);
+                        const bool first = c == 1;
+                        const int hs = c <= columns - 1 ? P_MATCH + (columns - 1 - c) * P_MATCH2 : 0;
+                        CellIn ci;
+                        ci.row = row; ci.c = c; ci.rows = rows; ci.insNeededBase = (columns - c) + 1;
+                        ci.cl1 = cl1; ci.ref1 = ref1; ci.refN = false; ci.gap = false; ci.match = cl1 == ref1; ci.act = inRange & started;
+                        ci.refPen = 0; ci.limitP = max(vlimP, max(T.minScoreOff - hs, floorv) + 2048); ci.floorP = floorP; ci.subfloor = subfloor;
+                        ci.dgM = first ? insPrev : T.M[i]; ci.dgD = first ? insPrev : T.D[i]; ci.dgI = first ? insPrev : T.I[i];
+                        ci.lM = first ? insRow : leftM; ci.lD = first ? insRow : leftD;
+                        ci.upM = i < 3 ? T.M[i + 1] : uM; ci.upI = i < 3 ? T.I[i + 1] : uI;
+                        ci.delForce = delForce;
+                        ci.insForce = ((rowOne & (c > 1)) | ((row > rows - 2) & (c < columns - 1))) ? INT_MAX : INT_MIN;
+                        ci.pm8 = ((T.mprev >> i) & 1) ? 8 : 0;
+                        const CellOut co = cell_update<Scheme11ts, false>(pen, ci);
+                        const bool good = co.goodM | co.goodD | co.goodI;
+                        goods |= good ? (1u << i) : 0u;
+                        mbits |= ci.match ? (1u << i) : 0u;
+                        word |= co.nib << (4 * i);
+                        T.M[i] = co.nM; T.D[i] = co.nD; T.I[i] = co.nI;
+                        leftM = co.nM; leftD = co.nD;
+                    }
+                    if (q == 0 && (goods & 1u) && c0 >= 1) T.bail = 1;
+                    if (q == Q - 1 && (goods & 8u) && c0 + 3 < columns) T.bail = 1;
+                    T.gprev = gIn; T.gmask = (int)goods; T.mprev = (int)mbits; T.gpass = (gIn | (goods ? 1 : 0));
+                    dir[((long long)row * 2 + T.slot) * 64 + lane] = word | (goods << 16);
+                }
+            }
+        }
+        asm volatile("s_waitcnt vmcnt(0)" ::: "memory");
+        __builtin_amdgcn_wave_barrier();
+
+#pragma unroll
+        for (int s = 0; s < 2; s++) {
+            const long long j = jobJ[s];
+            const int set = (q & 1) ^ s;
+            int lastM[4], lastD[4], lastI[4];
+#pragma unroll
+            for (int i = 0; i < 4; i++) { lastM[i] = set ? S[1].M[i] : S[0].M[i]; lastD[i] = set ? S[1].D[i] : S[0].D[i]; lastI[i] = set ? S[1].I[i] : S[0].I[i]; }
+            int bail = set ? S[1].bail : S[0].bail;
+            for (int d = 1; d < Q; d <<= 1) bail |= __shfl_xor(bail, d, 64);
+            const bool live = jobOk[s];
+            if (live && bail) { if (q == 0) { const unsigned k = atomicAdd(p.fast_count, 1u); p.fast_list[k] = (int)j; nLeft++; } }
+            if (!(live && !bail)) continue;
+
+            const bbmsa_job jb = p.jobs[j];
+            int a = jb.refStartLoc, b = jb.refEndLoc;
+            if (jb.flags & BBMSA_CLAMP_WINDOW) {
+                a = max(0, a); b = min(jb.ref_len - 1, b);
+                if (b - a >= p.maxColumns) b = min(jb.ref_len - 1, a + p.maxColumns - 1);
+            }
+            const int rows = jb.read_len, columns = b - a + 1, mode = jb.flags & BBMSA_MODE_MASK;
+            const int minScoreOff = (mode == BBMSA_FILL_LIMITED ? jb.minScore - 120 : jb.minScore) * 2048;
+            const int subfloor = minScoreOff - ((rows - 1) * P_MATCH2 + P_MATCH) - 5 * P_MATCH2;
+            const int D0 = (columns - rows) / 2 - B / 2;
+            const uint8_t *rdL = jobLds + (grp * 2 + s) * (RB + FB), *rfL = rdL + RB;
+            const unsigned *jdir = dir + s * 64 + groupBase;
+
+            const int per = (rows + Q - 1) / Q;
+            const int rFirst = q * per + 1, rLast = min(rows, (q + 1) * per);
+            int iters = 0, lastColStart = 1, lastHasGood = 0, lastEntered = 0;
+            {
+                unsigned long long pg = 0;
+                if (rFirst > 1 && rFirst <= rLast) for (int l = 0; l < Q; l++) pg |= (unsigned long long)((ld_coherent(jdir + (long long)(rFirst - 1) * 128 + l) >> 16) & 15u) << (4 * l);
+                for (int r = rFirst; r <= rLast; r++) {
+                    unsigned long long g = 0;
+                    for (int l = 0; l < Q; l++) g |= (unsigned long long)((ld_coherent(jdir + (long long)r * 128 + l) >> 16) & 15u) << (4 * l);
+                    const bool entered = r == 1 || pg != 0;
+                    const int colStart = r == 1 ? 1 : (r - 1) + D0 + __builtin_ctzll(pg | (1ull << 63));
+                    const int colStop = r == 1 ? columns : (r - 1) + D0 + (63 - __builtin_clzll(pg | 1ull));
+                    const int maxG = g ? r + D0 + (63 - __builtin_clzll(g)) : -2;
+                    const int endc = min(columns, max(colStop, maxG) + 1);
+                    if (entered) iters += endc - colStart + 1;
+                    if (r == rows) { lastColStart = colStart; lastHasGood = g != 0; lastEntered = entered; }
+                    pg = g;
+                }
+            }
+            for (int d = 1; d < Q; d <<= 1) iters += __shfl_xor(iters, d, 64);
+            {
+                const int owner = groupBase + (rows - 1) / per;
+                lastColStart = __shfl(lastColStart, owner, 64); lastHasGood = __shfl(lastHasGood, owner, 64); lastEntered = __shfl(lastEntered, owner, 64);
+            }
+            int bScore = INT_MIN, bKey = INT_MAX, bPacked = 0;
+#pragma unroll
+            for (int i = 0; i < 4; i++) {
+                const int c = rows + D0 + 4 * q + i;
+                if (c >= 1 && c <= columns) {
+                    const int v[3] = {lastM[i], lastD[i], lastI[i]};
+#pragma unroll
+                    for (int st = 0; st < 3; st++) {
+                        const int sc = v[st] & kScoreMask, key = st * 65536 + c;
+                        if (sc > bScore || (sc == bScore && key < bKey)) { bScore = sc; bKey = key; bPacked = v[st]; }
+                    }
+                }
+            }
+            for (int d = 1; d < Q; d <<= 1) {
+                const int os = __shfl_xor(bScore, d, 64), ok_ = __shfl_xor(bKey, d, 64), op = __shfl_xor(bPacked, d, 64);
+                if (os > bScore || (os == bScore && ok_ < bKey)) { bScore = os; bKey = ok_; bPacked = op; }
+            }
+            const int bCol = bKey & 65535, bState = bKey >> 16;
+
+            int res1, res2, res3, res4 = 0;
+            bool fillNull = false;
+            if (!lastEntered) { res1 = 1; res2 = 0; res3 = kBadOff; res4 = 1; fillNull = true; }
+            else if (!lastHasGood) { res1 = max(1, lastColStart - 1); res2 = 0; res3 = subfloor; res4 = 1; fillNull = true; }
+            else if (bScore < minScoreOff) { res1 = bCol; res2 = bState; res3 = bScore; res4 = 1; fillNull = true; }
+            else { res1 = bCol; res2 = bState; res3 = bScore >> kScoreOffset; }
+
+            const bool wantScore = !fillNull && (jb.flags & BBMSA_DO_SCORE);
+            const bool wantTrace = !fillNull && (jb.flags & BBMSA_DO_TRACEBACK) && p.match != nullptr;
+            int sc[8] = {0, 0, 0, 0, 0, 0, 0, 0};
+            int scoreLen = 0, matchLen = 0;
+            if (wantScore || wantTrace) {
+                uint8_t *out = p.match ? p.match + j * (long long)p.match_stride : nullptr;
+                auto nib_at = [&](int r, int c) -> unsigned {
+                    const int pos = c - r - D0;
+                    if (pos < 0 || pos >= B) return 0u;
+                    return (ld_coherent(jdir + (long long)r * 128 + (pos >> 2)) >> (4 * (pos & 3))) & 15u;
+                };
+                int row = rows, col = res1, state = res2, n = 0, stateTime = 0;
+                while (row > 0 && col > 0) {
+                    if (state == 0) {
+                        const int rr = row - q, cq = col - q;
+                        const bool inside = rr >= 1 && cq >= 1;
+                        const unsigned nibv = inside ? nib_at(rr, cq) : 0u;
+                        const bool brk = !inside || (nibv & 3u) != 0u;
+                        const unsigned long long mine = (__ballot(brk) >> groupBase) & ((1ull << Q) - 1ull);
+                        const int fb = mine ? __builtin_ctzll(mine) : Q;
+                        const int fbInside = __shfl((int)inside, groupBase + min(fb, Q - 1), 64);
+                        const int fbPrev = __shfl((int)(nibv & 3u), groupBase + min(fb, Q - 1), 64);
+                        const int consumed = (fb < Q && fbInside) ? fb + 1 : fb;
+                        if (wantTrace && q < consumed && n + q < p.match_stride) {
+                            const int cb = rdL[rr - 1], rb = rfL[min(max(cq - D0, 0), rows + B)];
+                            out[n + q] = (cb == rb) ? 'm' : ((!fully_defined(cb) || !fully_defined(rb)) ? 'N' : 'S');
+                        }
+                        stateTime += fb;
+                        if (fb < Q && fbInside) { stateTime = 0; state = fbPrev; }
+                        row -= consumed; col -= consumed; n += consumed;
+                    } else {
+                        const unsigned nibv = nib_at(row, col);
+                        int prev;
+                        uint8_t sym;
+                        if (state == 1) { prev = (nibv & 4u) ? 1 : 0; sym = 'D'; col--; }
+                        else { prev = (nibv & 8u) ? 2 : 0; sym = (col >= columns) ? 'Y' : 'I'; row--; }
+                        if (wantTrace && q == 0 && n < p.match_stride) out[n] = sym;
+                        n++;
+                        if (prev == state) stateTime++; else stateTime = 0;
+                        state = prev;
+                    }
+                }
+                int colS = col;
+                if (row > colS) colS -= row;
+                const int bestRefStart = a + colS, bestRefStop = a + res1 - 1;
+                int padLeft = 0, padRight = 0;
+                if (bestRefStart < a) padLeft = max(0, a - bestRefStart);
+                else if (bestRefStart == a && state == 2) padLeft = stateTime;
+                const int bW = (jb.flags & BBMSA_INTERNAL_GAPPED) ? jb.ref_len : b;
+                if (bestRefStop > bW) padRight = max(0, bestRefStop - bW);
+                else if (bestRefStop == bW && res2 == 2) padRight = bPacked & kTimeMask;
+                if (wantScore) {
+                    sc[0] = bScore >> kScoreOffset; sc[1] = bestRefStart; sc[2] = bestRefStop; sc[3] = rows; sc[4] = res1; sc[5] = res2;
+                    scoreLen = (padLeft > 0 || padRight > 0) ? 8 : 6;
+                    if (scoreLen == 8) { sc[6] = padLeft; sc[7] = padRight; }
+                }
+                if (wantTrace) {
+                    const int xs = (col != row) ? row : 0;
+                    for (int i = q; i < xs; i += Q) if (n + i < p.match_stride) out[n + i] = 'X';
+                    n += xs;
+                    if (n > p.match_stride) matchLen = -1;
+                    else {
+                        asm volatile("s_waitcnt vmcnt(0)" ::: "memory");
+                        __builtin_amdgcn_wave_barrier();
+                        for (int i = q; i < n / 2; i += Q) {
+                            const uint8_t lo = (uint8_t)ld_coherent(out + i), hi = (uint8_t)ld_coherent(out + n - 1 - i);
+                            out[i] = hi; out[n - 1 - i] = lo;
+                        }
+                        matchLen = n;
+                    }
+                }
+            }
+            if (q == 0) {
+                bbmsa_result r;
+                r.result[0] = rows; r.result[1] = res1; r.result[2] = res2; r.result[3] = res3; r.result[4] = res4;
+                r.status = (fillNull && mode == BBMSA_FILL_LIMITED) ? BBMSA_ST_NULL : BBMSA_ST_OK;
+                r.iterations = iters;
+#pragma unroll
+                for (int i = 0; i < 8; i++) r.score[i] = sc[i];
+                r.score_len = scoreLen; r.match_len = matchLen; r.fill_kind = 0; r.columns = columns;
+                p.results[j] = r;
+                nDone++;
+            }
+        }
+        __builtin_amdgcn_fence(__ATOMIC_ACQ_REL, "wavefront");
+        __builtin_amdgcn_wave_barrier();
+    }
+    if (p.stats) {
+        for (int d = 32; d >= 1; d >>= 1) { nDone += __shfl_xor(nDone, d, 64); nLeft += __shfl_xor(nLeft, d, 64); }
+        if (lane == 0) { if (nDone) atomicAdd(&p.stats[0], nDone); if (nLeft) atomicAdd(&p.stats[1], nLeft); }
+    }
+}
+
+template __global__ void msa_fill_band_kernel<8>(const NarrowParams);
+
+const void *band_kernel() { return (const void *)msa_fill_band_kernel<8>; }
+int band_lds_bytes(int tableLen, int bandRows) {
+    constexpr int Q = 8, B = 4 * Q, JOBS = 2 * (64 / Q);
+    const int RB = (bandRows + 4 + 3) & ~3, FB = (bandRows + B + 4 + 3) & ~3;
+    return lds_table_ints(tableLen) * 4 + 4 * JOBS * (RB + FB);
+}
+
+}
diff --git a/bbmap_amd/csrc/msa_fill_narrow.hip b/bbmap_amd/csrc/msa_fill_narrow.hip
--- a/bbmap_amd/csrc/msa_fill_narrow.hip
+++ /dev/null
@@ -1,379 +0,0 @@
-#include "msa_common.h"
-
-namespace bbmsa {
-
-namespace {
-
-constexpr int NB = 16;
-static_assert(NB == 16, "the sliding reference-byte window (w0/w1/w2) and the 64-bit direction word are laid out for 16 diagonals");
-
-__device__ inline int ctime_n(int t) { return t > kMaxTime ? kMaxTime - 3 : t; }
-__device__ inline int del_step_n(int streak) {
-    if (streak == 0) return P_DEL;
-    if (streak < 5) return P_DEL2;
-    if (streak < 20) return P_DEL3;
-    if (streak < 80) return P_DEL4;
-    return (streak & 3) == 0 ? P_DEL5 : 0;
-}
-__device__ inline int ins_step_n(int streak) {
-    if (streak == 0) return P_INS;
-    if (streak < 5) return P_INS2;
-    if (streak < 20) return P_INS3;
-    return P_INS4;
-}
-__device__ inline int sub_step_n(int streak) {
-    if (streak == 0) return P_SUB;
-    if (streak < 5) return P_SUB2;
-    return P_SUB3;
-}
-
-struct CellOut { int M, D, I; bool good; unsigned nib; };
-
-__device__ inline CellOut cell_eval(int row, int col, int rows, int columns, int call0, int call1, int ref0, int ref1,
-                                    int vlimit, int hlimit, int floorv, int subfloor,
-                                    int dM, int dD, int dI, int lM, int lD, int uM, int uI) {
-    CellOut o;
-    const bool gap = ref1 == '-';
-    const bool match = (call1 == ref1) & (ref1 != 'N');
-    const bool prevMatch = (call0 == ref0) & (ref0 != 'N');
-    const int limit = max(vlimit, hlimit);
-    const int limit3 = max(floorv, match ? limit - P_MATCH2 : limit - P_SUB3);
-    const int delNeeded = max(0, row - col - 1);
-    const int insNeeded = max(0, (rows - row) - (columns - col) - 1);
-    const int delPen = calc_del_off(delNeeded);
-    const int insPen = calc_ins_cum_off(insNeeded);
-    bool anyGood = false;
-    const int dm = dM & kScoreMask, dd = dD & kScoreMask, di = dI & kScoreMask;
-    const int lm = lM & kScoreMask, ld = lD & kScoreMask;
-    const int um = uM & kScoreMask, ui = uI & kScoreMask;
-
-    int timeM = 0;
-    if (gap | ((dm <= limit3) & (dd <= limit3) & (di <= limit3))) {
-        o.M = subfloor;
-    } else {
-        const int streak = dM & kTimeMask;
-        int a, bonus, tA;
-        if (match) { a = dm + (prevMatch ? P_MATCH2 : P_MATCH); bonus = P_MATCH; tA = prevMatch ? streak + 1 : 1; }
-        else {
-            if ((ref1 != 'N') & (call1 != 'N')) a = dm + (prevMatch ? (streak <= 1 ? P_SUBR : P_SUB) : sub_step_n(streak));
-            else a = dm;
-            bonus = P_SUB; tA = prevMatch ? 1 : streak + 1;
-        }
-        const int bb = dd + bonus, cc = di + bonus;
-        int score, time;
-        if ((a >= bb) & (a >= cc)) { score = a; time = tA; }
-        else if (bb >= cc) { score = bb; time = 1; }
-        else { score = cc; time = 1; }
-        const int limit2 = delNeeded > 0 ? limit - delPen : (insNeeded > 0 ? limit - insPen : limit);
-        if (score >= limit2) anyGood = true; else score = subfloor;
-        timeM = time;
-        o.M = score | ctime_n(time);
-    }
-    bool aWinsD = true;
-    if (((lm <= limit) & (ld <= limit)) | (row < 3) | (row > rows - 3)) {
-        o.D = subfloor;
-    } else {
-        const int streak = lD & kTimeMask;
-        int a = lm + P_DEL, bsc = ld + del_step_n(streak);
-        if (ref1 == 'N') { a += P_DEL_REF_N; bsc += P_DEL_REF_N; }
-        else if (gap) { a += P_GAP; bsc += P_GAP; }
-        int score, time;
-        if (a >= bsc) { score = a; time = 1; } else { score = bsc; time = streak + 1; aWinsD = false; }
-        int limit2 = limit;
-        if (insNeeded > 0) limit2 = limit - insPen;
-        else if (delNeeded > 0) limit2 = limit - calc_del_off(time + delNeeded) + calc_del_off(time);
-        if (score >= limit2) anyGood = true; else score = subfloor;
-        o.D = score | ctime_n(time);
-    }
-    bool aWinsI = true;
-    if (gap | ((um <= limit) & (ui <= limit)) | ((row < 2) & (col > 1)) | ((row > rows - 2) & (col < columns - 1))) {
-        o.I = subfloor;
-    } else {
-        const int streak = uI & kTimeMask;
-        const int a = um + P_INS, bsc = ui + ins_step_n(streak);
-        int score, time;
-        if (a >= bsc) { score = a; time = 1; } else { score = bsc; time = streak + 1; aWinsI = false; }
-        int limit2 = limit;
-        if (delNeeded > 0) limit2 = limit - delPen;
-        else if (insNeeded > 0) limit2 = limit - calc_ins_cum_off(time + insNeeded) + calc_ins_cum_off(time);
-        if (score >= limit2) anyGood = true; else score = subfloor;
-        o.I = score | ctime_n(time);
-    }
-    const bool msStay = (timeM > 1) | (dm >= max(dd, di));
-    const unsigned nibM = msStay ? 0u : ((dd >= di) ? 1u : 2u);
-    o.nib = nibM | (aWinsD ? 0u : 4u) | (aWinsI ? 0u : 8u);
-    o.good = anyGood;
-    return o;
-}
-
-}
-
-#ifndef BBMSA_NARROW_OCC
-#define BBMSA_NARROW_OCC 2
-#endif
-__global__ __launch_bounds__(64, BBMSA_NARROW_OCC) void msa_fill_narrow_kernel(const NarrowParams p) {
-    const int lane = threadIdx.x;
-    unsigned long long *dirw = p.dirbuf + (long long)blockIdx.x * (long long)(p.maxRows + 1) * 64;
-    const bool ctxBanded = !(p.bandwidth < 1 && p.bandwidthRatio <= 0.0f);
-    unsigned nDone = 0, nLeft = 0;
-    const long long NJ = job_count(p.njobs, p.njobs_dev);
-
-    for (;;) {
-        long long j = -1;
-        bbmsa_job jb;
-        jb.read_off = 0; jb.ref_off = 0; jb.read_len = 0; jb.ref_len = 0; jb.refStartLoc = 0; jb.refEndLoc = -1; jb.minScore = 0; jb.flags = 0;
-        int rows = 0, a = 0, b = -1, columns = 0, minScore = 0, mode = 0;
-        for (;;) {
-            const long long q = (long long)atomicAdd(p.queue, 1u);
-            if (q >= NJ) break;
-            const bbmsa_job t = p.jobs[q];
-            int ta = t.refStartLoc, tb = t.refEndLoc;
-            const int tmode = t.flags & BBMSA_MODE_MASK;
-            if (t.flags & BBMSA_CLAMP_WINDOW) {
-                ta = max(0, ta); tb = min(t.ref_len - 1, tb);
-                if (tb - ta >= p.maxColumns) tb = min(t.ref_len - 1, ta + p.maxColumns - 1);
-            }
-            const int trows = t.read_len, tcols = tb - ta + 1;
-            bool cand = !ctxBanded && trows >= NB && tcols >= trows && trows <= p.maxRows && tcols <= p.maxColumns &&
-                        tmode != BBMSA_FILL_UNLIMITED_RAW;
-            int tmin = t.minScore;
-            if (cand && tmode == BBMSA_FILL_LIMITED) {
-                if (tmin < 1 || (tcols + trows < 90) || (tcols > trows + min(170, trows + 20))) cand = false;
-                else tmin -= 120;
-            }
-            if (cand && (70 + 100 * (trows - 1)) - tmin > p.maxSlack) cand = false;
-            if (cand) { j = q; jb = t; rows = trows; a = ta; b = tb; columns = tcols; minScore = tmin; mode = tmode; break; }
-            const unsigned k = atomicAdd(p.fast_count, 1u);
-            p.fast_list[k] = (int)q;
-        }
-        if (!__any(j >= 0)) break;
-        bool active = j >= 0;
-        const uint8_t *rd = p.reads + jb.read_off;
-        const uint8_t *rf = p.refs + jb.ref_off + a;
-        const int D0 = (columns - rows) / 2 - NB / 2;
-
-        const int maxGain = (rows - 1) * P_MATCH2 + P_MATCH;
-        const int minScoreOff = minScore * 2048;
-        const int floorv = minScoreOff - maxGain;
-        const int subfloor = floorv - 5 * P_MATCH2;
-
-        int vs = 0;
-        if (active) {
-            bool allDef = true;
-            for (int c = 0; c < columns; c++) allDef = allDef && fully_defined(rf[c]);
-            bool nextDef = false;
-            for (int i = rows - 1; i >= 0; i--) {
-                const bool def = fully_defined(rd[i]);
-                vs += def ? (nextDef ? P_MATCH2 : P_MATCH) : 0;
-                nextDef = def;
-            }
-            if (!allDef) { active = false; const unsigned k = atomicAdd(p.fast_count, 1u); p.fast_list[k] = (int)j; nLeft++; }
-        }
-        auto hlimit_at = [&](int col) -> int {
-            const int hs = col <= columns - 1 ? P_MATCH + (columns - 1 - col) * P_MATCH2 : 0;
-            return max(minScoreOff - hs, floorv);
-        };
-
-        int aM[NB + 1], aD[NB + 1], aI[NB + 1];
-#pragma unroll
-        for (int i = 0; i <= NB; i++) { aM[i] = 0; aD[i] = 0; aI[i] = 0; }
-        long long iters = 0;
-        int prevMin = 1, prevMax = columns;
-        int stoppedRow = INT_MAX;
-        int lastColStart = 1, lastHasGood = 0;
-        int bestM = 0, bestD = 0, bestI = 0, bestMc = -1, bestDc = -1, bestIc = -1;
-        unsigned long long w0 = 0, w1 = 0, w2 = 0;
-        auto ref_col = [&](int c) -> unsigned { return (active && c >= 1 && c <= columns) ? (unsigned)rf[c - 1] : 0u; };
-        if (active) {
-            for (int k = 0; k < 8; k++) w0 |= (unsigned long long)ref_col(1 + D0 - 1 + k) << (8 * k);
-            for (int k = 0; k < 8; k++) w1 |= (unsigned long long)ref_col(1 + D0 - 1 + 8 + k) << (8 * k);
-            for (int k = 0; k < 2; k++) w2 |= (unsigned long long)ref_col(1 + D0 - 1 + 16 + k) << (8 * k);
-        }
-        int call0 = '?';
-        int maxRowsBatch = active ? rows : 0;
-        for (int d = 32; d >= 1; d >>= 1) maxRowsBatch = max(maxRowsBatch, __shfl_xor(maxRowsBatch, d, 64));
-
-        for (int row = 1; row <= maxRowsBatch; row++) {
-            const bool rowAct = active && row <= rows && stoppedRow == INT_MAX;
-            if (!__any(rowAct)) break;
-            int call1 = 0;
-            bool enter = false;
-            int colStart = 0, colStop = 0, vlimit = 0;
-            if (rowAct) {
-                call1 = rd[row - 1];
-                colStart = prevMin; colStop = prevMax;
-                enter = !(colStart < 0 || colStop < colStart);
-                if (!enter) stoppedRow = row;
-                const bool def = fully_defined(call1);
-                const bool nextDef = row < rows ? fully_defined(rd[row]) : false;
-                vs -= def ? (nextDef ? P_MATCH2 : P_MATCH) : 0;
-                vlimit = max(minScoreOff - vs, floorv);
-            }
-            const int c0 = row + D0;
-            bool go = rowAct && enter;
-            if (go && row == 1) {
-                bool outGood = false;
-                for (int c = 1; c <= columns; c++) {
-                    if (c >= c0 && c < c0 + NB) continue;
-                    const int ref1 = rf[c - 1], ref0 = c < 2 ? '!' : rf[c - 2];
-                    const CellOut o = cell_eval(1, c, rows, columns, call0, call1, ref0, ref1, vlimit, hlimit_at(c), floorv, subfloor,
-                                                0, 0, 0, c == 1 ? calc_ins_cum_off(1) : subfloor, c == 1 ? calc_ins_cum_off(1) : subfloor, 0, 0);
-                    outGood = outGood || o.good;
-                }
-                iters += (long long)(columns - max(0, min(columns, c0 + NB - 1) - max(1, c0) + 1));
-                if (outGood) go = false;
-            }
-            if (go && row > 1 && (colStart < c0 || colStart > c0 + NB - 1)) go = false;
-            const bool bailEarly = rowAct && enter && !go;
-            int minGood = -1, maxGood = -2;
-            bool rowDone = false;
-            int leftM = subfloor, leftD = subfloor;
-            if (go && colStart == 1) { leftM = calc_ins_cum_off(row); leftD = leftM; }
-            unsigned long long word = 0;
-            const int insPrev = calc_ins_cum_off(row - 1);
-            const bool lastRow = row == rows;
-#pragma unroll
-            for (int i = 0; i < NB; i++) {
-                const int c = c0 + i;
-                const bool inRow = go && c >= colStart && c >= 1 && c <= columns && !rowDone;
-                int nM = subfloor, nD = subfloor, nI = subfloor;
-                if (inRow) {
-                    const unsigned rb0 = (unsigned)((i < 8 ? (w0 >> (8 * (i & 7))) : (w1 >> (8 * (i & 7)))) & 255u);
-                    const int k1 = i + 1;
-                    const unsigned rb1 = (unsigned)((k1 < 8 ? (w0 >> (8 * (k1 & 7))) : (k1 < 16 ? (w1 >> (8 * (k1 & 7))) : (w2 >> (8 * (k1 & 7))))) & 255u);
-                    const int ref0 = c < 2 ? '!' : (int)rb0, ref1 = (int)rb1;
-                    const int dM = (c == 1) ? insPrev : aM[i], dD = (c == 1) ? insPrev : aD[i], dI = (c == 1) ? insPrev : aI[i];
-                    const int uM = (i + 1 < NB) ? aM[i + 1] : (row == 1 ? 0 : subfloor);
-                    const int uI = (i + 1 < NB) ? aI[i + 1] : (row == 1 ? 0 : subfloor);
-                    const CellOut o = cell_eval(row, c, rows, columns, call0, call1, ref0, ref1, vlimit, hlimit_at(c), floorv, subfloor,
-                                                dM, dD, dI, leftM, leftD, uM, uI);
-                    nM = o.M; nD = o.D; nI = o.I;
-                    iters++;
-                    if (o.good) { maxGood = c; if (minGood < 0) minGood = c; }
-                    if (c > colStop && maxGood < c) rowDone = true;
-                    word |= (unsigned long long)o.nib << (4 * i);
-                    if (lastRow) {
-                        if (bestMc < 0 || (nM & kScoreMask) > (bestM & kScoreMask)) { bestM = nM; bestMc = c; }
-                        if (bestDc < 0 || (nD & kScoreMask) > (bestD & kScoreMask)) { bestD = nD; bestDc = c; }
-                        if (bestIc < 0 || (nI & kScoreMask) > (bestI & kScoreMask)) { bestI = nI; bestIc = c; }
-                    }
-                    leftM = nM; leftD = nD;
-                }
-                if (rowAct) { aM[i] = nM; aD[i] = nD; aI[i] = nI; }
-            }
-            const bool unfinished = go && row > 1 && !rowDone && (c0 + NB - 1 < columns);
-            if (bailEarly || unfinished) {
-                active = false;
-                const unsigned k = atomicAdd(p.fast_count, 1u);
-                p.fast_list[k] = (int)j;
-                nLeft++;
-            } else if (go) {
-                prevMin = minGood; prevMax = maxGood;
-                dirw[(long long)row * 64 + lane] = word;
-                if (lastRow) { lastColStart = colStart; lastHasGood = minGood >= 0; }
-            }
-            {
-                const unsigned nb = ref_col(row + 1 + D0 - 1 + NB + 1);
-                w0 = (w0 >> 8) | (w1 << 56);
-                w1 = (w1 >> 8) | (w2 << 56);
-                w2 = (w2 >> 8) | ((unsigned long long)nb << 8);
-            }
-            call0 = call1;
-        }
-
-        int bScore = INT_MIN, bCol = -1, bState = 0, bPacked = 0;
-        if (bestMc >= 0) { bScore = bestM & kScoreMask; bCol = bestMc; bState = 0; bPacked = bestM; }
-        if (bestDc >= 0 && (bestD & kScoreMask) > bScore) { bScore = bestD & kScoreMask; bCol = bestDc; bState = 1; bPacked = bestD; }
-        if (bestIc >= 0 && (bestI & kScoreMask) > bScore) { bScore = bestI & kScoreMask; bCol = bestIc; bState = 2; bPacked = bestI; }
-        int res1, res2, res3, res4 = 0;
-        bool fillNull = false;
-        if (stoppedRow <= rows) { res1 = 1; res2 = 0; res3 = kBadOff; res4 = 1; fillNull = true; }
-        else if (!lastHasGood) { res1 = max(1, lastColStart - 1); res2 = 0; res3 = subfloor; res4 = 1; fillNull = true; }
-        else if (bScore < minScoreOff) { res1 = bCol; res2 = bState; res3 = bScore; res4 = 1; fillNull = true; }
-        else { res1 = bCol; res2 = bState; res3 = bScore >> kScoreOffset; }
-
-        asm volatile("s_waitcnt vmcnt(0)" ::: "memory");
-
-        if (active) {
-            bbmsa_result r;
-            r.result[0] = rows; r.result[1] = res1; r.result[2] = res2; r.result[3] = res3; r.result[4] = res4;
-            r.status = (fillNull && mode == BBMSA_FILL_LIMITED) ? BBMSA_ST_NULL : BBMSA_ST_OK;
-            r.iterations = iters;
-            for (int i = 0; i < 8; i++) r.score[i] = 0;
-            r.score_len = 0; r.match_len = 0; r.fill_kind = 0; r.columns = columns;
-            if (!fillNull && (jb.flags & (BBMSA_DO_SCORE | BBMSA_DO_TRACEBACK))) {
-                const bool wantTrace = (jb.flags & BBMSA_DO_TRACEBACK) && p.match != nullptr;
-                uint8_t *out = wantTrace ? p.match + j * (long long)p.match_stride : nullptr;
-                int row = rows, col = res1, state = res2, n = 0, gaps = 0, stateTime = 0;
-                bool overflow = false;
-                while (row > 0 && col > 0) {
-                    const int i = col - row - D0;
-                    unsigned nib = 0;
-                    if (i >= 0 && i < NB) nib = (unsigned)(__hip_atomic_load(&dirw[(long long)row * 64 + lane], __ATOMIC_RELAXED, __HIP_MEMORY_SCOPE_AGENT) >> (4 * i)) & 15u;
-                    int prev;
-                    uint8_t sym;
-                    if (state == 0) {
-                        prev = (int)(nib & 3u);
-                        const int cb = rd[row - 1], rb = rf[col - 1];
-                        sym = (cb == rb) ? 'm' : ((!fully_defined(cb) || !fully_defined(rb)) ? 'N' : 'S');
-                        row--; col--;
-                    } else if (state == 1) {
-                        prev = (nib & 4u) ? 1 : 0;
-                        const int rb = rf[col - 1];
-                        if (rb == '-') { sym = '-'; gaps++; } else sym = 'D';
-                        col--;
-                    } else {
-                        prev = (nib & 8u) ? 2 : 0;
-                        sym = (col >= columns) ? 'Y' : 'I';
-                        row--;
-                    }
-                    if (wantTrace) { if (n < p.match_stride) out[n] = sym; else overflow = true; }
-                    n++;
-                    if (state == prev) stateTime++; else stateTime = 0;
-                    state = prev;
-                }
-                if (jb.flags & BBMSA_DO_SCORE) {
-                    int colS = col;
-                    if (row > colS) colS -= row;
-                    const int bestRefStart = a + colS, bestRefStop = a + res1 - 1;
-                    int padLeft = 0, padRight = 0;
-                    if (bestRefStart < a) padLeft = max(0, a - bestRefStart);
-                    else if (bestRefStart == a && state == 2) padLeft = stateTime;
-                    const int bW = (jb.flags & BBMSA_INTERNAL_GAPPED) ? jb.ref_len : b;
-                    if (bestRefStop > bW) padRight = max(0, bestRefStop - bW);
-                    else if (bestRefStop == bW && res2 == 2) padRight = bPacked & kTimeMask;
-                    r.score[0] = bScore >> kScoreOffset; r.score[1] = bestRefStart; r.score[2] = bestRefStop;
-                    r.score[3] = rows; r.score[4] = res1; r.score[5] = res2;
-                    if (padLeft > 0 || padRight > 0) { r.score[6] = padLeft; r.score[7] = padRight; r.score_len = 8; }
-                    else r.score_len = 6;
-                }
-                if (wantTrace) {
-                    if (col != row) { while (row > 0) { if (n < p.match_stride) out[n] = 'X'; else overflow = true; n++; row--; col--; } }
-                    const bool keepGaps = (jb.flags & BBMSA_TRACE_KEEP_GAPS) != 0;
-                    const int totalLen = keepGaps ? n : n + gaps * (kGapLen - 1);
-                    if (overflow || totalLen > p.match_stride) r.match_len = -1;
-                    else {
-                        for (int x = 0, y = n - 1; x < y; x++, y--) { const uint8_t t0 = out[x]; out[x] = out[y]; out[y] = t0; }
-                        if (gaps > 0 && !keepGaps) {
-                            int w = totalLen - 1;
-                            for (int x = n - 1; x >= 0; x--) {
-                                const uint8_t ch = out[x];
-                                if (ch != '-') out[w--] = ch;
-                                else for (int g = 0; g < kGapLen; g++) out[w--] = 'D';
-                            }
-                        }
-                        r.match_len = totalLen;
-                    }
-                }
-            }
-            p.results[j] = r;
-            nDone++;
-        }
-    }
-    if (p.stats) {
-        for (int d = 32; d >= 1; d >>= 1) { nDone += __shfl_xor(nDone, d, 64); nLeft += __shfl_xor(nLeft, d, 64); }
-        if (lane == 0) { if (nDone) atomicAdd(&p.stats[0], nDone); if (nLeft) atomicAdd(&p.stats[1], nLeft); }
-    }
-}
-
-}
diff --git a/bbmap_amd/csrc/msa_host.hip b/bbmap_amd/csrc/msa_host.hip
--- a/bbmap_amd/csrc/msa_host.hip
+++ b/bbmap_amd/csrc/msa_host.hip
@@ -22,7 +22,8 @@
 int strip_pipe_sync_ints(int K);
 const void *fast_kernel_for(int R, bool banded);
 template <class S> __global__ void msa_fill_generic_kernel(const GenericParams p);
-__global__ void msa_fill_narrow_kernel(const NarrowParams p);
+const void *band_kernel();
+int band_lds_bytes(int tableLen, int bandRows);
 }
 
 namespace bbmsa {
@@ -223,11 +224,14 @@
     c->narrowSlack = env_int("BBMSA_NARROW_SLACK", 2000);
     if (!c->banded && env_int("BBMSA_NARROW", 1) != 0) {
         int perCU = 0;
-        BBHIP(hipOccupancyMaxActiveBlocksPerMultiprocessor(&perCU, (const void *)bbmsa::msa_fill_narrow_kernel, 64, 0));
+        c->bandRows = cfg->maxRows < 256 ? cfg->maxRows : 256;
+        c->bandLds = bbmsa::band_lds_bytes(c->tableLen, c->bandRows);
+        if (c->bandLds > 64 * 1024) BBHIP(hipFuncSetAttribute(bbmsa::band_kernel(), hipFuncAttributeMaxDynamicSharedMemorySize, c->bandLds));
+        BBHIP(hipOccupancyMaxActiveBlocksPerMultiprocessor(&perCU, bbmsa::band_kernel(), 256, c->bandLds));
         if (perCU < 1) perCU = 1;
-        if (perCU > 16) perCU = 16;
+        if (perCU > 4) perCU = 4;
         c->narrowBlocks = c->numCUs * perCU;
-        BBHIP(hipMalloc(&c->d_narrowDir, (size_t)c->narrowBlocks * (size_t)(cfg->maxRows + 1) * 64 * 8));
+        BBHIP(hipMalloc(&c->d_bandDir, (size_t)c->narrowBlocks * 4 * (size_t)(c->bandRows + 1) * 128 * 4));
     }
     c->sortByWidth = env_int("BBMSA_SORT_BY_WIDTH", 0) != 0;
     { const int lat = env_int("BBMSA_LATENCY_JOBS", 0); if (lat > 0) BBTRY(bbmsa_set_latency_jobs(c, lat)); }
@@ -248,7 +252,7 @@
     if (c->d_matrix) (void)hipFree(c->d_matrix);
     if (c->d_limits) (void)hipFree(c->d_limits);
     if (c->d_wideDir) (void)hipFree(c->d_wideDir);
-    if (c->d_narrowDir) (void)hipFree(c->d_narrowDir);
+    if (c->d_bandDir) (void)hipFree(c->d_bandDir);
     if (c->d_stripBoundary) (void)hipFree(c->d_stripBoundary);
     if (c->d_stripTmp) (void)hipFree(c->d_stripTmp);
     if (c->d_pipeBoundary) (void)hipFree(c->d_pipeBoundary);
@@ -344,11 +348,12 @@
         bbmsa::NarrowParams np;
         set_batch(np, c, B);
         np.queue = c->d_counters + 3; np.fast_list = fastList; np.fast_count = c->d_counters + 4;
-        np.dirbuf = c->d_narrowDir; np.stats = c->d_counters + 5; np.maxSlack = c->narrowSlack;
+        np.stats = c->d_counters + 5; np.maxSlack = c->narrowSlack;
+        np.dirbuf32 = c->d_bandDir; np.tableLen = c->tableLen; np.bandRows = c->bandRows;
         long long nb = (n_jobs + 63) / 64;
         if (nb > c->narrowBlocks) nb = c->narrowBlocks;
-        hipLaunchKernelGGL(bbmsa::msa_fill_narrow_kernel, dim3((unsigned)nb), dim3(64), 0, stream, np);
-        BBHIP(hipGetLastError());
+        void *nargs[] = {&np};
+        BBHIP(hipLaunchKernel(bbmsa::band_kernel(), dim3((unsigned)nb), dim3(256), nargs, (size_t)c->bandLds, stream));
     }
     if (sortJobs) {
         if (!c->d_widthHist) BBHIP(hipMalloc(&c->d_widthHist, bbmsa::WIDTH_BUCKETS * 4));
```

After: 9.492 million (median of 6 runs). 1.05x the previous value.
